# jcmgray/cotengra

Hardware: AMD Instinct MI355X
Metric: contracted FLOP/s (whole node), Sycamore n53 m20 sliced amplitude (higher is better)
Workload: dtype complex64; 1 GPU; Sycamore n53 m20 amplitude, sliced tree, one slice per step per GPU; network=examples/benchmarks/sycamore_n53_m20_s0_e0_pABCDCDAB.json, tree=sycamore_m20_native.json, width_log2=32, parallelism=slice-parallel x1, 1 RCCL reduce, arithmetic=fp16x2 stem pairs and long tiled steps + fp32 MFMA

## Files before the change

### cotengra_amd/csrc/ctg_common.h

```cpp
#pragma once

#include <hip/hip_runtime.h>
#include <cstdlib>
#include <type_traits>
#include <stdint.h>

namespace ctg {

inline bool env_on(const char* name) {
    const char* v = getenv(name);
    return v != nullptr && v[0] != '\0' && !(v[0] == '0' && v[1] == '\0');
}
inline int env_state(const char* name) { return getenv(name) == nullptr ? -1 : (env_on(name) ? 1 : 0); }

inline hipError_t lds_opt_in(const void* kern, int bytes, unsigned long long* done) {
    int dev = 0;
    hipError_t e = hipGetDevice(&dev);
    if (e != hipSuccess) return e;
    const unsigned long long bit = 1ull << (dev & 63);
    if (__atomic_load_n(done, __ATOMIC_ACQUIRE) & bit) return hipSuccess;
    e = hipFuncSetAttribute(kern, hipFuncAttributeMaxDynamicSharedMemorySize, bytes);
    if (e != hipSuccess) {
        (void)hipGetLastError();
        return e;
// ... 58 lines not shown
    void* C;
    const int64_t* soffA;
    const int64_t* soffB;
    const int64_t* soffC;
    int64_t R;
    int64_t Bt;
    int64_t K;
    int64_t N;
    int64_t row_lo;
    int32_t row_lo_shift;
    RowTab rowA, rowB, rowC;
    int64_t k_lo;
    int64_t k_hi_len;
    int32_t k_lo_shift;
    RowTab kA, kB;
    const int64_t* nB;
    const int64_t* nC;
    const int64_t* bA;
    const int64_t* bB;
    const int64_t* bC;
    const double* facA;
    const double* facB;
    int32_t check_zero;
    int32_t nz, z0;
    uint64_t row_lo_magic, k_lo_magic;
    int64_t scratch_total;
    int64_t zA, zB, zC;
    int64_t zsA, zsB, zsC;
    int32_t zqA, zqB;
    int32_t bf3;
};

struct StemArgs {
    const void* A;
    const void* B1;
    const void* B2;
    void* C;
    const int64_t* soffA;
    const int64_t* soffB1;
    const int64_t* soffB2;
    const int64_t* soffC;
    int32_t K1, N1, K2, N2;
    int32_t nr1;
    int32_t rows2;
    int32_t ng2;
    int32_t ld2;
    int64_t n_tiles, g_lo;
    int32_t g_lo_shift;
    int32_t check_zero;
    int32_t vec;
    int32_t bf3;
    const int64_t* gA_hi;
    const int64_t* gA_lo;
    const int64_t* gC_hi;
    const int64_t* gC_lo;
    const int64_t* kj_a;
    const int64_t* lane_a;
    const int64_t* rt_a;
    const int64_t* chunk_a;
    const int64_t* b1_off;
    const int64_t* b2_off;
    const int64_t* mid_row;
    const int64_t* mid_col;
    const int64_t* out_row;
    const int64_t* out_col;
    const double* facA;
    const double* facB1;
    const double* facB2;
    int32_t nz, z0;
    int64_t zA, zB1, zB2, zC;
    int64_t zsA, zsB1, zsB2, zsC;
    int32_t one;
    int32_t tri, KM, NM, rowsM, ngM, ldM;
    const void* BM;
    const int64_t* soffBM;
    const int64_t* bm_off;
    const int64_t* mid2_row;
    const int64_t* mid2_col;
    const double* facBM;
    int64_t zBM, zsBM;
    int64_t a_elems, c_elems;
    const float* amax;
    float* cmax;
};

__device__ __forceinline__ int64_t zid(const StepArgs& p) { return (int64_t)p.z0 + blockIdx.y; }
constexpr int kMaxSub = 16;
__device__ __forceinline__ void record_max(float* slot, float v) {
    atomicMax((unsigned*)slot + ((blockIdx.x + (threadIdx.x >> 6)) & (kMaxSub - 1)), __builtin_bit_cast(unsigned, v));
}
__device__ __forceinline__ float read_max(const float* slot) {
    float m = slot[0];
#pragma unroll
    for (int i = 1; i < kMaxSub; ++i) m = fmaxf(m, slot[i]);
    return m;
}
__device__ __forceinline__ int64_t zgroup(int64_t z, int32_t q) { return q > 1 ? z / q * q : z; }
__device__ __forceinline__ int64_t zoffA(const StepArgs& p) { const int64_t z = zgroup(zid(p), p.zqA); return p.soffA[z * p.zsA] + z * p.zA; }
__device__ __forceinline__ int64_t zoffB(const StepArgs& p) { const int64_t z = zgroup(zid(p), p.zqB); return p.soffB[z * p.zsB] + z * p.zB; }
__device__ __forceinline__ int64_t zoffC(const StepArgs& p) { const int64_t z = zid(p); return p.soffC[z * p.zsC] + z * p.zC; }

__device__ __forceinline__ double step_alpha(const StepArgs& p) {
    if (p.facA == nullptr) return 1.0;
    const double f = (*p.facA) * (*p.facB);
    if (f == 0.0 && p.check_zero) return 0.0;
    return 1.0 / f;
}

template <int I, int N, typename F>
__device__ __forceinline__ void static_for(F&& f) {
    if constexpr (I < N) {
        f(std::integral_constant<int, I>{});
        static_for<I + 1, N>(f);
    }
}

__device__ __forceinline__ int64_t uniform64(int64_t v) {
    const unsigned lo = __builtin_amdgcn_readfirstlane((unsigned)(v & 0xffffffffll));
    const unsigned hi = __builtin_amdgcn_readfirstlane((unsigned)((unsigned long long)v >> 32));
    return (int64_t)(((unsigned long long)hi << 32) | lo);
}

__device__ __forceinline__ float dpp_swap1(float v) {
    return __builtin_bit_cast(float, __builtin_amdgcn_mov_dpp(__builtin_bit_cast(int, v), 0xB1, 0xF, 0xF, true));
}
__device__ __forceinline__ float2 pair_rows(float a_t, float a_t1, bool odd) {
    const float x = dpp_swap1(a_t), y = dpp_swap1(a_t1);
    float2 v;
    v.x = odd ? y : a_t;
    v.y = odd ? a_t1 : x;
    return v;
}
__device__ __forceinline__ float2 pair_rows(float a_t, float a_t1, bool odd, float alpha) {
    const float x = dpp_swap1(a_t), y = dpp_swap1(a_t1);
    float2 v;
    v.x = (odd ? y : a_t) * alpha;
    v.y = (odd ? a_t1 : x) * alpha;
    return v;
}

__device__ __forceinline__ int64_t sload64(const int64_t* p) {
    typedef const int64_t __attribute__((address_space(4))) * cptr;
    return *(cptr)(uintptr_t)p;
}

__device__ __forceinline__ int64_t zoffA_s(const StepArgs& p) { const int64_t z = zgroup(zid(p), p.zqA); return sload64(p.soffA + z * p.zsA) + z * p.zA; }
__device__ __forceinline__ int64_t zoffB_s(const StepArgs& p) { const int64_t z = zgroup(zid(p), p.zqB); return sload64(p.soffB + z * p.zsB) + z * p.zB; }
__device__ __forceinline__ int64_t zoffC_s(const StepArgs& p) { const int64_t z = zid(p); return sload64(p.soffC + z * p.zsC) + z * p.zC; }

__device__ __forceinline__ void split_k(const StepArgs& p, int64_t k, int64_t& hi, int64_t& lo) {
    if (p.k_lo_shift >= 0) {
        hi = k >> p.k_lo_shift;
        lo = k & (p.k_lo - 1);
    } else if (p.k_lo_magic != 0) {
        hi = (int64_t)__umul64hi((uint64_t)k, p.k_lo_magic);
        lo = k - hi * p.k_lo;
    } else {
        hi = k / p.k_lo;
        lo = k - hi * p.k_lo;
    }
}

__device__ __forceinline__ void split_row(const StepArgs& p, int64_t i, int64_t& hi, int64_t& lo) {
    if (p.row_lo_shift >= 0) {
        hi = i >> p.row_lo_shift;
        lo = i & (p.row_lo - 1);
// ... 126 lines not shown

template <typename F>
inline hipError_t for_each_z(const StepArgs& p, F launch_one) {
    if (p.nz <= 1) return launch_one(p);
    for (int z = 0; z < p.nz; ++z) {
        StepArgs q = p;
        q.z0 = p.z0 + z;
        q.nz = 1;
        const hipError_t e = launch_one(q);
        if (e != hipSuccess) return e;
    }
    return hipSuccess;
}

template <typename F>
inline hipError_t for_each_z_chunk(const StepArgs& p, int64_t fit, F launch_chunk) {
    if (fit < 1) fit = 1;
    for (int64_t z = 0; z < p.nz; z += fit) {
        StepArgs q = p;
        q.z0 = p.z0 + (int32_t)z;
        q.nz = (int32_t)(p.nz - z < fit ? p.nz - z : fit);
        const hipError_t e = launch_chunk(q);
        if (e != hipSuccess) return e;
    }
    return hipSuccess;
}


hipError_t launch_pair_valu(int dtype, const StepArgs& p, void* scratch, int64_t scratch_bytes,
                            hipStream_t stream);
struct ValuGroupItem {
    StepArgs p;
    int64_t col_tiles, n_tiles;
    int32_t tn_shift;
    uint32_t block_begin, n_blocks;
};
constexpr int64_t kValuGroupMaxTiles = 4096;
bool valu_thread_per_output(const StepArgs& p);
void pair_valu_name(int dtype, const StepArgs& p, int64_t scratch_bytes, char* buf, size_t n);
uint32_t valu_group_fill(const StepArgs& p, ValuGroupItem* it, uint32_t block_begin);
hipError_t launch_pair_valu_group(int dtype, const ValuGroupItem* d_items, int n_items, uint32_t blocks,
                                  int nz, hipStream_t stream);
hipError_t launch_pair_mfma(int dtype, const StepArgs& p, const MfmaHints& h, void* scratch,
                            int64_t scratch_bytes, hipStream_t stream);
constexpr int64_t kPickKredMinK = 1 << 15, kPickKredMaxM = 512;
inline bool pick_route_kred(int64_t M, int64_t K) { return K >= kPickKredMinK && M <= kPickKredMaxM; }
hipError_t launch_pair_pick(int dtype, const StepArgs& p, int vec, void* scratch, int64_t scratch_bytes,
                            hipStream_t stream);
void pair_pick_name(int dtype, const StepArgs& p, int vec, int64_t scratch_bytes, char* buf, size_t n);
constexpr int64_t kPickRowsMfmaMinRowLo = 32, kPickRowsMfmaMinN = 8, kPickRowsMfmaMinK = 8;
inline bool pick_rows_route_mfma(int64_t row_lo, int64_t K, int64_t N, int dtype) {
    return dtype == 2 && row_lo >= kPickRowsMfmaMinRowLo && N >= kPickRowsMfmaMinN && K >= kPickRowsMfmaMinK;
}
hipError_t launch_pair_pick_rows(int dtype, const StepArgs& p, int vec, int b_fixed, hipStream_t stream);
void pair_pick_rows_name(int dtype, const StepArgs& p, int vec, int b_fixed, char* buf, size_t n);
struct FastGroupItem {
    StepArgs p;
    MfmaHints h;
    int64_t tiles_m, tiles_n;
    uint32_t block_begin, n_blocks;
};
constexpr int64_t kFastGroupMaxTiles = 128;
int fast_group_key(const StepArgs& p, const MfmaHints& h);
uint32_t fast_group_fill(const StepArgs& p, const MfmaHints& h, FastGroupItem* it, uint32_t block_begin);
hipError_t launch_pair_mfma_fast_group(int key, const FastGroupItem* d_items, int n_items, uint32_t blocks,
                                       int nz, hipStream_t stream);
bool rowwise_ok(const StepArgs& p);
void pair_mfma_c64_name(const StepArgs& p, const MfmaHints& h, int64_t scratch_bytes, char* buf, size_t n);
int64_t fast_lane_table_bytes();
hipError_t launch_fast_lane_consts(const StepArgs& p, const MfmaHints& h, void* out, hipStream_t stream);
hipError_t launch_pair_mfma_c128(const StepArgs& p, int flags, hipStream_t stream);
void pair_mfma_c128_name(const StepArgs& p, char* buf, size_t n);
hipError_t launch_pair_mfma_real(int dtype, const StepArgs& p, int flags, hipStream_t stream);
void pair_mfma_real_name(int dtype, const StepArgs& p, int flags, char* buf, size_t n);
bool stem2_supported(const StemArgs& p);
bool stem3_supported(const StemArgs& p);
hipError_t launch_stem2(const StemArgs& p, hipStream_t stream);
void stem2_kernel_name(const StemArgs& p, char* buf, size_t n);
bool stem2h_supported(const StemArgs& p);
bool stem2h_uses_h2(const StemArgs& p);
bool stem2_uses_bf3(const StemArgs& p);
hipError_t launch_stem2h(const StemArgs& p, hipStream_t stream);
void stem2h_kernel_name(const StemArgs& p, char* buf, size_t n);

hipError_t launch_single(int dtype, const StepArgs& p, hipStream_t stream);
bool pair_bf16x3_on(const StepArgs& p);
hipError_t launch_accum(int dtype, const StepArgs& p, const StripState* st, void* wide, const double* inscale, int leaf,
                        hipStream_t stream);
struct AccumGroupItem {
    StepArgs p;
    void* wide;
    int32_t leaf;
    uint32_t block_begin, n_blocks;
};
constexpr int64_t kAccumGroupMaxBlocks = 1 << 16;
uint32_t accum_group_fill(const StepArgs& p, void* wide, int leaf, AccumGroupItem* it, uint32_t block_begin);
hipError_t launch_accum_group(int dtype, const AccumGroupItem* d_items, int n_items, uint32_t blocks, int nz,
                              const double* inscale, hipStream_t stream);
hipError_t launch_prescale_inputs(int dtype, void* inputs, const int64_t* offs, const int64_t* sizes, int64_t n_inputs,
                                  int* shift_total, double* inscale, hipStream_t stream);
hipError_t launch_narrow(int dtype, void* result, const void* wide, int64_t n, hipStream_t stream);
hipError_t launch_widen(int dtype, void* wide, const void* result, int64_t n, hipStream_t stream);

hipError_t launch_maxabs(int dtype, const void* x, int64_t n, double* fac, hipStream_t stream);
hipError_t launch_strip_prepare(const double* fac, const int32_t* counted, int64_t n_steps,
                                int64_t root_step, int check_zero, StripState* st, const double* inscale, hipStream_t stream);
hipError_t launch_rescale(int dtype, void* result, int64_t n, const StripState* st, hipStream_t stream);

struct SliceMeta {
    int64_t n_leaves;
    int64_t n_sliced;
    const int64_t* sizes;
    const int64_t* fixed;
    const int64_t* strides;
    double* fac;
    const int32_t* fac_zero;
    int64_t n_fac;
    float* smax;
    const int32_t* smax_zero;
    int64_t n_smax;
};
hipError_t launch_prologue(const SliceMeta& m, int64_t* state, int64_t* soff, int64_t sid,
                           hipStream_t stream, int nz = 1, int64_t stride = 1, const int64_t* ids = nullptr);
hipError_t launch_set_state(int64_t* state, int64_t next, int64_t stride, hipStream_t stream);

}
```

### cotengra_amd/csrc/ctg_exec_state.h

```cpp
#pragma once

#include <string>
#include <vector>

#include "../../include/ctg_hip.h"
#include "ctg_common.h"
#include "ctg_lds.h"

struct ctg_plan {
    int dtype = 0;
    int64_t n_inputs = 0;
    std::vector<int64_t> input_sizes, input_offsets;
    int64_t inputs_elems = 0, arena_elems = 0, result_elems = 0;
    int64_t n_steps = 0;
    std::vector<int64_t> steps;
    std::vector<int64_t> tables;
    int64_t n_sliced = 0;
    std::vector<int64_t> slice_sizes, slice_fixed, slice_strides;
    std::vector<int64_t> slice_group;
    bool has_groups = false;
    int64_t nslices = 1;
    std::vector<int64_t> max_soff;
};

struct ctg_exec {
    const ctg_plan* plan = nullptr;
    int device = 0;
    hipStream_t stream = nullptr;
    char* d_inputs = nullptr;
    char* d_arena = nullptr;
    char* d_result = nullptr;
    bool owns_result = false;
    char* d_wide = nullptr;
    int64_t* d_in_tab = nullptr;
    double* d_inscale = nullptr;
    int64_t* d_tables = nullptr;
    int64_t* d_misc = nullptr;
    int64_t* d_state = nullptr;
    int64_t* d_zero = nullptr;
    int64_t* d_soff = nullptr;
    void* d_scratch = nullptr;
    ctg::SliceMeta meta{};
    std::vector<ctg::StepArgs> args;
    std::vector<ctg::StemArgs> stem_args;
    int stem_bf16x3 = 1;
    int stem_arith = 2;
    float* d_stem_max = nullptr;
    int32_t* d_smax_zero = nullptr;
    float* smax_slot(int bank, int64_t s, int64_t z) const {
        return d_stem_max + (((int64_t)bank * plan_steps + s) * (batch > 1 ? batch : 1) + z) * ctg::kMaxSub;
    }
    ctg::SliceMeta meta_resetting(int which) const {
        ctg::SliceMeta m = meta;
        if (m.smax) m.smax_zero = d_smax_zero + (int64_t)which * m.n_smax;
        return m;
    }
    int64_t plan_steps = 0;
    std::vector<char> rec_wanted;
    std::vector<char> wave_member;
    std::vector<char> stem_h2_ran;
    std::vector<ctg::MfmaHints> hints;
    std::vector<ctg::MfmaHints> hints_b;
    uint16_t* d_ord_b = nullptr;
    char* d_lane_b = nullptr;
    uint16_t* d_ord = nullptr;
    char* d_lane = nullptr;
    int batch = 1;
    int group_d = 0;
    int64_t* d_batch_ids = nullptr;
    int64_t* h_ids = nullptr;
    size_t h_ids_cap = 0;
    hipEvent_t ev_ids = nullptr;
    int batch_nominal = 1;
    int64_t scratch_total = 0;
    struct Issue {
        int64_t step;
        int cls;
        int32_t item0, n;
        uint32_t blocks;
        bool shared = false;
    };
    std::vector<Issue> issue;
    std::vector<Issue> issue_reuse;
    std::vector<int32_t> lds_comp_of;
    int lds_first[2] = {0, 0}, lds_count[2] = {0, 0}, lds_bytes[2] = {0, 0};
    ctg::LdsCompDev* d_lds_comps = nullptr;
    char* d_lds_blob = nullptr;
    ctg::ValuGroupItem* d_group_items = nullptr;
    ctg::AccumGroupItem* d_accum_items = nullptr;
    std::vector<char> accum_member;
    ctg::FastGroupItem* d_fast_items = nullptr;
    std::vector<hipEvent_t> events;
    hipStream_t gstream = nullptr;
    hipGraphExec_t gexec = nullptr;
    hipEvent_t ev_in = nullptr, ev_out = nullptr;
    bool warm = false;
    bool soff_static = false;
    bool graph_off = false;
    int strip = 0, check_zero = 0;
    double* d_fac = nullptr;
    int32_t* d_counted = nullptr;
    int32_t* d_fac_zero = nullptr;
    std::vector<char> invariant;
    bool invariants_ready = false;
    std::vector<char> grouped;
    int64_t group_key = -1;
    ctg::StripState* d_strip = nullptr;
    int64_t root_step = -1;
    void* d_sample_blocks = nullptr;
    void* d_sample_io = nullptr;
    int64_t sample_blocks_bytes = 0, sample_io_bytes = 0;
    double sample_last[4] = {0, 0, 0, 0};
    float sample_pass_ms[2] = {0, 0};
    bool sample_last_valid = false;
    hipEvent_t sample_ev[3] = {nullptr, nullptr, nullptr};
    void* d_range = nullptr;
    int64_t range_bytes = 0;
    void* d_reduce = nullptr;
    int64_t reduce_bytes = 0;
};


inline int64_t ctg_item_size(int dtype) {
    static const int64_t k[4] = {4, 8, 8, 16};
    return k[dtype];
}

extern "C" __attribute__((visibility("hidden"))) void ctg_set_error_(const char* msg);

namespace ctg {
hipError_t launch_maxabs_f32(const void* base, const int64_t* soff, int64_t z, int64_t zs, int64_t zstride, int64_t n,
                             float* out, hipStream_t stream, int nz = 1, int out_zs = 0);
}

namespace ctg {
constexpr int64_t kRangeMaxBlocks = 2048;
constexpr int64_t kRangeMaxComponents = 1ll << 40;
int64_t range_blocks(int64_t n);
int64_t range_partial_bytes(int64_t blocks);
hipError_t launch_range_hist(const void* x, int64_t n, void* partials, int64_t blocks, int64_t* row, double* sumsq,
                             hipStream_t stream);
}
// ... 22 lines not shown
```

### cotengra_amd/csrc/ctg_runtime.hip

```cpp
#include <algorithm>
#include <cstdarg>
#include <cmath>
#include <cstdio>
#include <cstdlib>
#include <cstring>
#include <string>
#include <vector>

#include "ctg_exec_state.h"

using namespace ctg;

namespace {

thread_local std::string g_err;

int fail(int code, const char* fmt, ...) {
    char buf[1024];
    va_list ap;
    va_start(ap, fmt);
    vsnprintf(buf, sizeof(buf), fmt, ap);
    va_end(ap);
    g_err = buf;
    return code;
// ... 72 lines not shown
        return fail(CTG_E_INVALID, "step %lld: bad stem grid", sl);
    const int64_t rows1 = 1ll << nr1;
    const int64_t len[ST_COUNT] = {n_tiles / g_lo, g_lo, n_tiles / g_lo, g_lo, 8, 64, rows1 / 32, K1 / 16,
                                   K1 * N1, one ? 1 : K2 * N2, one ? 1 : rows1, one ? 1 : N1,
                                   one ? rows1 : rows2, one ? N1 : N2};
    int64_t mx[ST_COUNT], mn[ST_COUNT];
    for (int t = 0; t < ST_COUNT; ++t) {
        if (!tab_ok(p, h[SW_TABS + t], len[t]))
            return fail(CTG_E_BOUNDS, "step %lld: stem table outside the blob", sl);
        mx[t] = tab_max(p, h[SW_TABS + t], len[t], &mn[t]);
        if (mn[t] < 0) return fail(CTG_E_BOUNDS, "step %lld: negative stem offset", sl);
    }
    if (mx[ST_LANE_A] >= (1ll << 29))
        return fail(CTG_E_INVALID, "step %lld: stem lane offsets beyond 32 bits", sl);
    if (h[SW_VEC] != 0 && h[SW_VEC] != 1) return fail(CTG_E_INVALID, "step %lld: bad stem gather mode", sl);
    if (h[SW_VEC]) {
        const int64_t* kj = &p->tables[h[SW_TABS + ST_KJ_A]];
        for (int q = 0; q < 4; ++q)
            if (kj[2 * q + 1] != kj[2 * q] + 1 || (kj[2 * q] & 1))
                return fail(CTG_E_INVALID, "step %lld: stem slots not paired for 16-byte gathers", sl);
        const int odd_tabs[5] = {ST_GA_HI, ST_GA_LO, ST_LANE_A, ST_RT_A, ST_CHUNK_A};
        for (int t : odd_tabs)
            for (int64_t i = 0; i < len[t]; ++i)
                if (p->tables[h[SW_TABS + t] + i] & 1)
                    return fail(CTG_E_INVALID, "step %lld: odd stem offset under 16-byte gathers", sl);
        if ((r[W_A_OFF] & 1) || r[W_A_LEAF] >= 0)
            return fail(CTG_E_INVALID, "step %lld: stem operand not aligned for 16-byte gathers", sl);
    }
    if (h[SW_TRI] != 0 && h[SW_TRI] != 1) return fail(CTG_E_INVALID, "step %lld: bad stem stage count", sl);
    const bool tri = h[SW_TRI] == 1;
    int64_t bm_top = 0;
    if (tri) {
        const int64_t KM = h[SW_KM], NM = h[SW_NM], rowsM = h[SW_ROWSM];
        if (one || KM < 16 || KM > 128 || NM < 16 || NM > 128 || rowsM < 32 || rowsM > (1 << 16) ||
            h[SW_LDM] != KM + 4 || rows1 * N1 != rowsM * KM || rowsM * NM != rows2 * K2)
            return fail(CTG_E_INVALID, "step %lld: three-step tile shape the kernel does not take", sl);
        a.tri = 1; a.KM = (int)KM; a.NM = (int)NM; a.rowsM = (int)rowsM; a.ngM = (int)h[SW_NGM]; a.ldM = (int)h[SW_LDM];
        a.vec = (int)h[SW_VEC];
        if (!stem3_supported(a))
            return fail(CTG_E_INVALID, "step %lld: three-step tile shape the kernel does not take", sl);
        const int64_t lenm[3] = {KM * NM, rowsM, NM};
        int64_t mxm[3], mnm[3];
        for (int t = 0; t < 3; ++t) {
            if (!tab_ok(p, h[SW_TABS_M + t], lenm[t]))
                return fail(CTG_E_BOUNDS, "step %lld: stem table outside the blob", sl);
            mxm[t] = tab_max(p, h[SW_TABS_M + t], lenm[t], &mnm[t]);
            if (mnm[t] < 0) return fail(CTG_E_BOUNDS, "step %lld: negative stem offset", sl);
        }
        bm_top = mxm[0];
        if (mx[ST_MID_ROW] + mx[ST_MID_COL] >= rowsM * (KM + 4) || mxm[1] + mxm[2] >= rows2 * (K2 + 4))
            return fail(CTG_E_BOUNDS, "step %lld: intermediate tile overflows its LDS", sl);
        const int64_t cap = space_elems(p, h[SW_BM_SPACE]);
        if (cap < 0) return fail(CTG_E_INVALID, "step %lld: bad space", sl);
        if (h[SW_BM_LEAF] < -1 || h[SW_BM_LEAF] > p->n_inputs) return fail(CTG_E_INVALID, "step %lld: bad leaf", sl);
        const int64_t hi = h[SW_BM_OFF] + (h[SW_BM_LEAF] >= 0 ? p->max_soff[h[SW_BM_LEAF]] : 0) + bm_top;
        if (h[SW_BM_OFF] < 0 || hi >= cap)
            return fail(CTG_E_BOUNDS, "step %lld: stem operand m reaches element %lld of a space of %lld", sl,
                        (long long)hi, (long long)cap);
    }
    if (!one && !tri && mx[ST_MID_ROW] + mx[ST_MID_COL] >= rows2 * (K2 + 4))
        return fail(CTG_E_BOUNDS, "step %lld: intermediate tile overflows its LDS", sl);
    struct Op { int64_t space, off, leaf, size, top; char name; };
    const Op ops[4] = {
        {r[W_A_SPACE], r[W_A_OFF], r[W_A_LEAF], r[W_A_SIZE],
         mx[ST_GA_HI] + mx[ST_GA_LO] + mx[ST_RT_A] + mx[ST_CHUNK_A] + mx[ST_KJ_A] + mx[ST_LANE_A], 'A'},
        {r[W_B_SPACE], r[W_B_OFF], r[W_B_LEAF], r[W_B_SIZE], mx[ST_B1_OFF], 'B'},
        {h[SW_B2_SPACE], h[SW_B2_OFF], h[SW_B2_LEAF], h[SW_B2_SIZE], mx[ST_B2_OFF], 'b'},
        {r[W_C_SPACE], r[W_C_OFF], r[W_C_LEAF], r[W_C_SIZE],
         mx[ST_GC_HI] + mx[ST_GC_LO] + mx[ST_OUT_ROW] + mx[ST_OUT_COL], 'C'},
    };
    for (const Op& op : ops) {
        if (one && op.name == 'b') continue;
        const int64_t cap = space_elems(p, op.space);
        if (cap < 0) return fail(CTG_E_INVALID, "step %lld: bad space", sl);
        if (op.leaf < -1 || op.leaf > p->n_inputs) return fail(CTG_E_INVALID, "step %lld: bad leaf", sl);
        if (op.name == 'C' && op.space == SPACE_INPUTS)
            return fail(CTG_E_INVALID, "step %lld: writes into the inputs space", sl);
        const int64_t hi = op.off + (op.leaf >= 0 ? p->max_soff[op.leaf] : 0) + op.top;
        if (op.off < 0 || hi >= cap)
            return fail(CTG_E_BOUNDS, "step %lld: stem operand %c reaches element %lld of a space of %lld",
                        sl, op.name, (long long)hi, (long long)cap);
    }
    return CTG_OK;
}

int validate_plan(ctg_plan* p) {
    if (p->dtype < 0 || p->dtype > 3) return fail(CTG_E_INVALID, "bad dtype %d", p->dtype);
    if (p->n_inputs < 1) return fail(CTG_E_INVALID, "plan needs at least one input");
    for (int64_t i = 0; i < p->n_inputs; ++i) {
        if (p->input_sizes[i] < 1 || p->input_offsets[i] < 0 ||
            p->input_offsets[i] + p->input_sizes[i] > p->inputs_elems)
            return fail(CTG_E_BOUNDS, "input %lld does not fit the inputs space", (long long)i);
    }
    p->nslices = 1;
    p->max_soff.assign(p->n_inputs + 1, 0);
    for (int64_t j = 0; j < p->n_sliced; ++j) {
        const int64_t d = p->slice_sizes[j], f = p->slice_fixed[j];
        if (d < 1) return fail(CTG_E_INVALID, "bad slice size");
        if (f >= 0 && d != 1) return fail(CTG_E_INVALID, "projected index must have size 1");
        p->nslices = (p->nslices > INT64_MAX / d) ? INT64_MAX : p->nslices * d;
        for (int64_t l = 0; l <= p->n_inputs; ++l) {
            const int64_t st = p->slice_strides[l * p->n_sliced + j];
            if (st < 0) return fail(CTG_E_INVALID, "negative slice stride");
            p->max_soff[l] += st * (f >= 0 ? f : d - 1);
        }
    }
    bool any_group = false;
    for (int64_t j = 0; j < p->n_sliced; ++j) {
        const int64_t g = p->slice_group[j];
        if (g != 0 && g != 1) return fail(CTG_E_INVALID, "bad slice group flag");
        if (g == 1 && p->slice_fixed[j] >= 0) return fail(CTG_E_INVALID, "a projected index cannot be a group index");
        any_group = any_group || g == 1;
    }
    p->has_groups = false;
    for (int64_t s = 0; s < p->n_steps; ++s) {
        const int64_t* r = &p->steps[s * STEP_WORDS];
        const int64_t kind = r[W_KIND];
        if (kind < 0 || kind > 3) return fail(CTG_E_INVALID, "step %lld: bad kind", (long long)s);
        if (r[W_INVARIANT] < 0 || r[W_INVARIANT] > 2 || (r[W_INVARIANT] == 2 && !any_group))
            return fail(CTG_E_INVALID, "step %lld: bad sharing class", (long long)s);
        p->has_groups = p->has_groups || (r[W_INVARIANT] == 2 && kind != KIND_ACCUM);
        if (kind == KIND_STEM2) {
            const int rc = validate_stem(p, s);
            if (rc != CTG_OK) return rc;
            continue;
        }
        if (r[W_KERNEL] < 0 || r[W_KERNEL] > 3)
            return fail(CTG_E_INVALID, "step %lld: bad kernel", (long long)s);
        if (r[W_KERNEL] == KERNEL_PICK_ROWS && (kind != KIND_PAIR || r[W_BT] != 1))
            return fail(CTG_E_INVALID, "step %lld: the pick rows kernel executes pair steps with Bt = 1 only", (long long)s);
        if (r[W_KERNEL] == KERNEL_PICK_ROWS)
            for (int w : {W_ROWA_HI, W_ROWA_LO, W_ROWB_HI, W_ROWB_LO, W_ROWC_HI, W_ROWC_LO, W_KA_HI, W_KA, W_KB_HI,
                          W_KB, W_NB, W_NC})
                if (r[w] < 0)
                    return fail(CTG_E_INVALID, "step %lld: the pick rows kernel needs every row, k and n table", (long long)s);
        if (r[W_KERNEL] == KERNEL_PICK && (kind != KIND_PAIR || r[W_N] != 1 || r[W_BT] != 1 || r[W_ROW_LO] != 1))
            return fail(CTG_E_INVALID, "step %lld: the pick kernel executes pair steps with N = 1, Bt = 1 and row_lo = 1 only",
                        (long long)s);
        if (r[W_KERNEL] == KERNEL_PICK)
            for (int w : {W_ROWA_HI, W_ROWA_LO, W_ROWB_HI, W_ROWB_LO, W_ROWC_HI, W_ROWC_LO, W_KA_HI, W_KA, W_KB_HI,
                          W_KB, W_NB, W_NC})
                if (r[w] < 0)
                    return fail(CTG_E_INVALID, "step %lld: the pick kernel needs every row, k and n table", (long long)s);
        if (r[W_KERNEL] == KERNEL_MFMA && kind != KIND_PAIR)
            return fail(CTG_E_INVALID, "step %lld: the matrix-core kernels execute pair steps only",
                        (long long)s);
        const int64_t R = r[W_R], Bt = r[W_BT], K = r[W_K], N = r[W_N];
        const int64_t row_lo = r[W_ROW_LO], row_hi = r[W_ROW_HI_LEN];
        const int64_t k_lo = r[W_K_LO], k_hi = r[W_K_HI_LEN];
        if (R < 1 || Bt < 1 || K < 1 || N < 1 || row_lo < 1 || row_hi < 1 || k_lo < 1 || k_hi < 1)
            return fail(CTG_E_INVALID, "step %lld: non-positive extent", (long long)s);
        if (row_lo * row_hi != R) return fail(CTG_E_INVALID, "step %lld: row split != R", (long long)s);
        if (k_lo * k_hi != K) return fail(CTG_E_INVALID, "step %lld: k split != K", (long long)s);
        if (r[W_KERNEL] == KERNEL_MFMA && Bt > 65535)
            return fail(CTG_E_INVALID, "step %lld: MFMA batch too large", (long long)s);

        struct Op { int space_w, off_w, leaf_w, size_w; int64_t rhi, rlo, khi, klo, n, b; bool used; };
        const bool pair = kind == KIND_PAIR, mfma = r[W_KERNEL] == KERNEL_MFMA;
        Op ops[3] = {
            {W_A_SPACE, W_A_OFF, W_A_LEAF, W_A_SIZE, r[W_ROWA_HI], r[W_ROWA_LO],
             kind != KIND_ACCUM ? r[W_KA_HI] : -1, kind != KIND_ACCUM ? r[W_KA] : -1, -1,
             mfma ? r[W_BA] : -1, true},
            {W_B_SPACE, W_B_OFF, W_B_LEAF, W_B_SIZE, mfma ? -1 : r[W_ROWB_HI], mfma ? -1 : r[W_ROWB_LO],
             r[W_KB_HI], r[W_KB], r[W_NB], mfma ? r[W_BB] : -1, pair},
            {W_C_SPACE, W_C_OFF, W_C_LEAF, W_C_SIZE, r[W_ROWC_HI], r[W_ROWC_LO], -1, -1,
             pair ? r[W_NC] : -1, mfma ? r[W_BC] : -1, true},
// ... 164 lines not shown
        auto magic = [](int64_t d, int64_t range) -> uint64_t {
            if (d < 2 || (d & (d - 1)) == 0 || range + 4096 >= (1ll << 32)) return 0;
            return (uint64_t)(~0ull / (uint64_t)d) + 1;
        };
        a.row_lo_magic = magic(a.row_lo, r[W_R]);
        a.rowA = RowTab{tab(W_ROWA_HI), tab(W_ROWA_LO)};
        a.rowB = RowTab{tab(W_ROWB_HI), tab(W_ROWB_LO)};
        a.rowC = RowTab{tab(W_ROWC_HI), tab(W_ROWC_LO)};
        a.k_lo = r[W_K_LO];
        a.k_hi_len = r[W_K_HI_LEN];
        a.k_lo_shift = log2_exact(a.k_lo);
        a.k_lo_magic = magic(a.k_lo, r[W_K]);
        a.kA = RowTab{tab(W_KA_HI), tab(W_KA)};
        a.kB = RowTab{tab(W_KB_HI), tab(W_KB)};
        a.nB = tab(W_NB);
        a.nC = tab(W_NC);
        a.bA = tab(W_BA);
        a.bB = tab(W_BB);
        a.bC = tab(W_BC);
        a.nz = 1;
        a.z0 = 0;
        a.scratch_total = e->scratch_total;
        a.zA = per_slice(r[W_A_SPACE], r[W_A_OFF]);
        a.zB = per_slice(r[W_B_SPACE], r[W_B_OFF]);
        a.zC = per_slice(r[W_C_SPACE], r[W_C_OFF]);
        a.zsA = r[W_A_LEAF] >= 0 ? p->n_inputs + 1 : 0;
        a.zsB = r[W_B_LEAF] >= 0 ? p->n_inputs + 1 : 0;
        a.zsC = r[W_C_LEAF] >= 0 ? p->n_inputs + 1 : 0;
        if (e->group_d > 1) {
            auto shared = [&](int64_t st) {
                return st >= 0 && st < p->n_steps && p->steps[st * STEP_WORDS + W_INVARIANT] == 2 &&
                       p->steps[st * STEP_WORDS + W_KIND] != KIND_ACCUM;
            };
            const int64_t d = e->group_d;
            if (shared(s)) {
                a.zA *= d; a.zB *= d; a.zC *= d;
                a.zsA *= d; a.zsB *= d; a.zsC *= d;
            } else if (r[W_KIND] == KIND_PAIR || r[W_KIND] == KIND_SINGLE) {
                auto writer = [&](int sw, int ow) -> int64_t {
                    if (r[sw] != SPACE_ARENA) return -1;
                    for (int64_t t = s - 1; t >= 0; --t) {
                        const int64_t* w = &p->steps[t * STEP_WORDS];
                        if (w[W_KIND] != KIND_ACCUM && w[W_C_SPACE] == SPACE_ARENA && w[W_C_OFF] == r[ow]) return t;
                    }
                    return -1;
                };
                if (shared(writer(W_A_SPACE, W_A_OFF))) a.zqA = (int32_t)d;
                if (r[W_KIND] == KIND_PAIR && shared(writer(W_B_SPACE, W_B_OFF))) a.zqB = (int32_t)d;
            }
        }
        a.facA = a.facB = nullptr;
        a.check_zero = e->check_zero;
        a.bf3 = e->stem_bf16x3;
        if (e->strip && r[W_KIND] == KIND_PAIR) {
            auto fac = [&](int w) -> const double* {
                return (r[w] >= 0 && r[w] < p->n_steps) ? e->d_fac + r[w] : e->d_fac + p->n_steps;
            };
            a.facA = fac(W_A_PROD);
            a.facB = fac(W_B_PROD);
        }
        if (r[W_KIND] == KIND_STEM2) {
            const int64_t* h = &p->tables[r[W_STEM]];
            StemArgs& q = e->stem_args[s];
            memset(&q, 0, sizeof(q));
            q.A = a.A;
            q.B1 = a.B;
            q.C = a.C;
            q.one = h[SW_ONE] == 1 ? 1 : 0;
            q.B2 = q.one ? nullptr : (char*)space_ptr(e, h[SW_B2_SPACE]) + h[SW_B2_OFF] * isz;
            q.soffA = a.soffA;
            q.soffB1 = a.soffB;
            q.soffC = a.soffC;
            q.soffB2 = h[SW_B2_LEAF] >= 0 ? e->d_soff + h[SW_B2_LEAF] : e->d_zero;
            q.K1 = (int)h[SW_K1]; q.N1 = (int)h[SW_N1]; q.K2 = (int)h[SW_K2]; q.N2 = (int)h[SW_N2];
            q.nr1 = (int)h[SW_NR1]; q.rows2 = (int)h[SW_ROWS2]; q.ng2 = (int)h[SW_NG2]; q.ld2 = (int)h[SW_LD2];
            q.n_tiles = h[SW_NTILES];
            q.g_lo = h[SW_GLO];
            q.g_lo_shift = log2_exact(q.g_lo);
            q.check_zero = e->check_zero;
            q.vec = (int)h[SW_VEC];
            q.bf3 = e->stem_bf16x3;
            q.a_elems = r[W_A_SIZE];
            q.c_elems = r[W_C_SIZE];
            const int64_t** tabs[ST_COUNT] = {&q.gA_hi, &q.gA_lo, &q.gC_hi, &q.gC_lo, &q.kj_a, &q.lane_a, &q.rt_a,
                                              &q.chunk_a, &q.b1_off, &q.b2_off, &q.mid_row, &q.mid_col,
                                              &q.out_row, &q.out_col};
            for (int t = 0; t < ST_COUNT; ++t) *tabs[t] = T + h[SW_TABS + t];
            q.nz = 1;
            q.z0 = 0;
            q.zA = a.zA; q.zB1 = a.zB; q.zC = a.zC;
            q.zB2 = per_slice(h[SW_B2_SPACE], h[SW_B2_OFF]);
            q.zsA = a.zsA; q.zsB1 = a.zsB; q.zsC = a.zsC;
            q.zsB2 = h[SW_B2_LEAF] >= 0 ? p->n_inputs + 1 : 0;
            if (e->strip) {
                auto fac = [&](int64_t w) -> const double* {
                    return (w >= 0 && w < p->n_steps) ? e->d_fac + w : e->d_fac + p->n_steps;
                };
                q.facA = fac(r[W_A_PROD]);
                q.facB1 = fac(r[W_B_PROD]);
                q.facB2 = q.one ? e->d_fac + p->n_steps : fac(h[SW_B2_PROD]);
                q.facBM = h[SW_TRI] == 1 ? fac(h[SW_BM_PROD]) : e->d_fac + p->n_steps;
            }
            if (h[SW_TRI] == 1) {
                q.tri = 1;
                q.KM = (int)h[SW_KM]; q.NM = (int)h[SW_NM]; q.rowsM = (int)h[SW_ROWSM]; q.ngM = (int)h[SW_NGM];
                q.ldM = (int)h[SW_LDM];
                q.BM = (char*)space_ptr(e, h[SW_BM_SPACE]) + h[SW_BM_OFF] * isz;
                q.soffBM = h[SW_BM_LEAF] >= 0 ? e->d_soff + h[SW_BM_LEAF] : e->d_zero;
                q.bm_off = T + h[SW_TABS_M];
                q.mid2_row = T + h[SW_TABS_M + 1];
                q.mid2_col = T + h[SW_TABS_M + 2];
                q.zBM = per_slice(h[SW_BM_SPACE], h[SW_BM_OFF]);
                q.zsBM = h[SW_BM_LEAF] >= 0 ? p->n_inputs + 1 : 0;
            }
        }
    }
}


int64_t tab2(const ctg_plan* p, int64_t hi_w, int64_t lo_w, int64_t lo_size, int64_t i) {
    return p->tables[hi_w + i / lo_size] + p->tables[lo_w + i % lo_size];
}

bool tile_additive(const ctg_plan* p, int64_t lo_w, int64_t lo_size, int64_t total, int B) {
    if (total % B) return false;
    if (lo_size % B) return false;
    for (int64_t t = 0; t < lo_size / B; ++t)
        for (int r = 0; r < B; ++r)
            if (p->tables[lo_w + t * B + r] - p->tables[lo_w + t * B] != p->tables[lo_w + r])
                return false;
    return true;
}

bool all_even(const ctg_plan* p, int64_t w, int64_t len, int64_t stride = 1) {
    for (int64_t i = 0; i < len; i += stride)
        if (p->tables[w + i] & 1) return false;
    return true;
}

bool pick_vec_ok(const ctg_plan* p, const int64_t* r) {
    const int64_t k_lo = r[W_K_LO];
    if ((k_lo & 1) || (r[W_A_OFF] & 1) || (r[W_B_OFF] & 1)) return false;
    for (int64_t i = 0; i < k_lo; ++i)
        if (p->tables[r[W_KA] + i] != i || p->tables[r[W_KB] + i] != i) return false;
    if (!all_even(p, r[W_KA_HI], r[W_K_HI_LEN]) || !all_even(p, r[W_KB_HI], r[W_K_HI_LEN])) return false;
    if (!all_even(p, r[W_ROWA_HI], r[W_ROW_HI_LEN]) || !all_even(p, r[W_ROWB_HI], r[W_ROW_HI_LEN])) return false;
    if (!all_even(p, r[W_ROWA_LO], r[W_ROW_LO]) || !all_even(p, r[W_ROWB_LO], r[W_ROW_LO]) || !all_even(p, r[W_NB], r[W_N]))
        return false;
    if (p->arena_elems & 1) return false;
    for (int lw : {W_A_LEAF, W_B_LEAF})
        if (r[lw] >= 0)
            for (int64_t j = 0; j < p->n_sliced; ++j)
                if (p->slice_strides[r[lw] * p->n_sliced + j] & 1) return false;
    return true;
}

void build_mfma_order(const ctg_plan* p, const int64_t* r, int bn, int BM,
                      std::vector<uint16_t>& blob, size_t* offA, size_t* offB, int* vecA,
                      int TB = 256) {
    const int BK = MFMA_BK;
    const int T = BM == 32 ? 64 : 256;
    const int64_t R = r[W_R], K = r[W_K], N = r[W_N];
    const int64_t BIG = INT64_MAX / 4;
    {
        const int n_el = BM * BK, per_t = n_el / T;
        std::vector<int64_t> off(n_el);
// ... 454 lines not shown
    if (ev1) (void)hipEventDestroy(ev1);
}

static bool tiled16_step(const ctg_exec* e, int64_t s) {
    const ctg_plan* p = e->plan;
    const int64_t* r = &p->steps[s * STEP_WORDS];
    if (r[W_KIND] != KIND_PAIR || r[W_KERNEL] != KERNEL_MFMA || p->dtype != CTG_C64) return false;
    const MfmaHints& h = e->hints[s];
    return !h.stream && h.fast && h.bf3 && e->stem_arith != 0 && !e->strip && e->d_stem_max != nullptr &&
           pair_bf16x3_on(e->args[s]);
}

static bool stem_step_h2(const ctg_exec* e, int64_t s, bool recorded) {
    return e->stem_arith == 2 && !e->strip && e->d_stem_max != nullptr && (recorded || env_on("CTG_STEM_H2_ALL")) &&
           stem2h_uses_h2(e->stem_args[s]) && env_state("CTG_STEM_H2") != 0;
}
static bool pair_step_h2(const ctg_exec* e, bool single) {
    return e->stem_arith == 2 && single && env_state("CTG_PAIR_H2") != 0;
}

static bool pair_records(const ctg_exec* e, int64_t s) {
    const ctg_plan* p = e->plan;
    const int64_t* r = &p->steps[s * STEP_WORDS];
    if (r[W_KIND] != KIND_PAIR || r[W_KERNEL] != KERNEL_MFMA || p->dtype != CTG_C64) return false;
    if (e->stem_arith == 0 || e->strip || e->d_stem_max == nullptr || e->grouped[s]) return false;
    const MfmaHints& h = e->hints[s];
    if (tiled16_step(e, s)) return h.splitk <= 1 && e->args[s].zqA <= 1 && e->args[s].zqB <= 1;
    if (e->stem_arith != 2 || e->wave_member[s] || !e->rec_wanted[s]) return false;
    return h.stream == 1 || (!h.stream && h.fast && !h.bf3 && h.splitk <= 1);
}

int launch_step(ctg_exec* e, int64_t s, hipStream_t stream) {
    const ctg_plan* p = e->plan;
    const int64_t* r = &p->steps[s * STEP_WORDS];
    hipError_t err = hipSuccess;
    if (!e->d_scratch && step_needs_scratch(e, s)) {
        const int rc = ensure_scratch(e);
        if (rc != CTG_OK) return rc;
    }
    switch (r[W_KIND]) {
        case KIND_SINGLE: err = launch_single(p->dtype, e->args[s], stream); break;
        case KIND_ACCUM:
            if (e->strip) {
                err = launch_strip_prepare(e->d_fac, e->d_counted, p->n_steps, e->root_step,
                                           e->check_zero, e->d_strip, e->d_inscale, stream);
                if (err == hipSuccess)
                    err = launch_rescale(p->dtype, e->d_result, p->result_elems, e->d_strip, stream);
                if (err == hipSuccess && e->d_wide)
                    err = launch_rescale(p->dtype + 1, e->d_wide, p->result_elems, e->d_strip, stream);
                if (err == hipSuccess) err = launch_accum(p->dtype, e->args[s], e->d_strip, wide_of_step(e, s), nullptr, -1, stream);
            } else {
                err = launch_accum(p->dtype, e->args[s], nullptr, wide_of_step(e, s), e->d_inscale, accum_leaf(p, s), stream);
            }
            break;
        case KIND_STEM2: {
            const int nz = e->args[s].nz;
            const bool rec = e->stem_arith != 0 && !e->strip && e->d_stem_max != nullptr;
            const int64_t prod = r[W_A_PROD];
            const bool prod_rec = prod >= 0 && prod < p->n_steps && e->stem_h2_ran[prod];
            const bool h2 = stem_step_h2(e, s, prod_rec);
            const bool records = h2 || (rec && stem2_uses_bf3(e->stem_args[s]));
            e->stem_h2_ran[s] = records ? 1 : 0;
            if (env_on("CTG_STEM_DEBUG"))
                fprintf(stderr, "stem step %lld: arith %d rec %d prod %lld prod_rec %d uses_h2 %d uses_bf3 %d -> h2 %d records %d\n",
                        (long long)s, e->stem_arith, (int)rec, (long long)prod, (int)prod_rec, (int)stem2h_uses_h2(e->stem_args[s]),
                        (int)stem2_uses_bf3(e->stem_args[s]), (int)h2, (int)records);
            for (int z = 0; z < nz && err == hipSuccess; ++z) {
                StemArgs q = e->stem_args[s];
                q.z0 = e->args[s].z0 + z;
                q.nz = 1;
                const int64_t zc = (e->invariant[s] || e->grouped[s]) ? 0 : q.z0;
                const int64_t za = (prod_rec && (e->invariant[prod] || e->grouped[prod])) ? 0 : q.z0;
                q.amax = h2 ? e->smax_slot(0, prod_rec ? prod : 0, za) : nullptr;
                q.cmax = records ? e->smax_slot(0, s, zc) : nullptr;
                if (h2 && !prod_rec) {
                    float* slot = e->smax_slot(1, s, q.z0);
                    err = hipMemsetAsync(slot, 0, sizeof(float) * kMaxSub, stream);
                    if (err == hipSuccess)
                        err = r[W_A_LEAF] >= 0 ? launch_maxabs_f32(q.A, nullptr, 0, 0, 0, q.a_elems, slot, stream)
                                               : launch_maxabs_f32(q.A, q.soffA, q.z0, q.zsA, q.zA, q.a_elems, slot, stream);
                    q.amax = slot;
                }
                if (err == hipSuccess) err = h2 ? launch_stem2h(q, stream) : launch_stem2(q, stream);
            }
            break;
        }
        case KIND_PAIR:
            if (r[W_KERNEL] == KERNEL_MFMA && p->dtype == CTG_C128)
                err = launch_pair_mfma_c128(e->args[s], e->hints[s].vecA , stream);
            else if (r[W_KERNEL] == KERNEL_MFMA && p->dtype != CTG_C64)
                err = launch_pair_mfma_real(p->dtype, e->args[s], e->hints[s].vecA, stream);
            else if (r[W_KERNEL] == KERNEL_MFMA) {
                const MfmaHints& h0 = (e->args[s].nz > 1 && !e->hints_b.empty()) ? e->hints_b[s] : e->hints[s];
                const bool tiled16 = tiled16_step(e, s) && !h0.stream && h0.fast && h0.bf3;
                if (tiled16) {
                    MfmaHints h = h0;
                    const StepArgs& a = e->args[s];
                    const bool single = h0.splitk <= 1 && a.zqA <= 1 && a.zqB <= 1 && !e->grouped[s] &&
                                        a.z0 + a.nz <= std::max(e->batch, 1);
                    const bool h2 = pair_step_h2(e, single);
                    h.h2 = h2 ? 1 : 0;
                    h.cmax = single ? e->smax_slot(0, s, 0) : nullptr;
                    h.cmax_zs = e->invariant[s] ? 0 : 1;
                    e->stem_h2_ran[s] = single ? 1 : 0;
                    for (int side = 0; side < 2 && h2 && err == hipSuccess; ++side) {
                        const int64_t prod = r[side == 0 ? W_A_PROD : W_B_PROD];
                        const float* mx = nullptr;
                        int zs = 1;
                        if (prod >= 0 && prod < p->n_steps && e->stem_h2_ran[prod] && !e->grouped[prod]) {
                            mx = e->smax_slot(0, prod, 0);
                            zs = e->invariant[prod] ? 0 : 1;
                        } else if (r[side == 0 ? W_A_LEAF : W_B_LEAF] >= 0) {
                            float* slot = e->smax_slot(1 + side, s, 0);
                            err = hipMemsetAsync(slot, 0, sizeof(float) * kMaxSub, stream);
                            if (err == hipSuccess)
                                err = launch_maxabs_f32(side == 0 ? a.A : a.B, nullptr, 0, 0, 0, r[side == 0 ? W_A_SIZE : W_B_SIZE], slot, stream);
                            mx = slot;
                            zs = 0;
                        } else {
                            float* slot = e->smax_slot(1 + side, s, 0);
                            float* at = slot + (int64_t)a.z0 * kMaxSub;
                            err = hipMemsetAsync(at, 0, sizeof(float) * kMaxSub * (size_t)a.nz, stream);
                            if (err == hipSuccess)
                                err = side == 0 ? launch_maxabs_f32(a.A, a.soffA, a.z0, a.zsA, a.zA, r[W_A_SIZE], at, stream, a.nz, kMaxSub)
                                                : launch_maxabs_f32(a.B, a.soffB, a.z0, a.zsB, a.zB, r[W_B_SIZE], at, stream, a.nz, kMaxSub);
                            mx = slot;
                        }
                        (side == 0 ? h.amax : h.bmax) = mx;
                        (side == 0 ? h.amax_zs : h.bmax_zs) = zs;
                    }
                    if (env_on("CTG_STEM_DEBUG"))
                        fprintf(stderr, "tiled step %lld: arith %d single %d -> h2 %d records %d (A prod %lld, B prod %lld)\n",
                                (long long)s, e->stem_arith, (int)single, (int)h2, (int)single, (long long)r[W_A_PROD],
                                (long long)r[W_B_PROD]);
                    if (err == hipSuccess) err = launch_pair_mfma(p->dtype, e->args[s], h, e->d_scratch, kScratchBytes, stream);
                } else {
                    const StepArgs& a = e->args[s];
                    const bool can = e->stem_arith == 2 && !e->strip && e->d_stem_max != nullptr && !e->grouped[s] &&
                                     !env_on("CTG_NO_PAIR_RECORD") &&
                                     !e->wave_member[s] && e->rec_wanted[s] && a.z0 + a.nz <= std::max(e->batch, 1) &&
                                     ((h0.stream == 1) || (!h0.stream && h0.fast && !h0.bf3 && h0.splitk <= 1));
                    if (!e->stem_h2_ran.empty()) e->stem_h2_ran[s] = can ? 1 : 0;
                    if (can) {
                        MfmaHints h = h0;
                        h.cmax = e->smax_slot(0, s, 0);
                        h.cmax_zs = e->invariant[s] ? 0 : 1;
                        err = launch_pair_mfma(p->dtype, a, h, e->d_scratch, kScratchBytes, stream);
                    } else {
                        err = launch_pair_mfma(p->dtype, a, h0, e->d_scratch, kScratchBytes, stream);
                    }
                }
            } else if (r[W_KERNEL] == KERNEL_PICK)
                err = launch_pair_pick(p->dtype, e->args[s], e->hints[s].vecA, e->d_scratch, kScratchBytes, stream);
            else if (r[W_KERNEL] == KERNEL_PICK_ROWS)
                err = launch_pair_pick_rows(p->dtype, e->args[s], e->hints[s].vecA, e->hints[s].fast, stream);
            else
                err = launch_pair_valu(p->dtype, e->args[s], e->d_scratch, kScratchBytes, stream);
            break;
    }
    if (err == hipSuccess && e->strip && (r[W_KIND] == KIND_PAIR || r[W_KIND] == KIND_STEM2)) {
        const char* c = (const char*)space_ptr(e, r[W_C_SPACE]) + r[W_C_OFF] * kItemSize[p->dtype];
        err = launch_maxabs(p->dtype, c, r[W_C_SIZE], e->d_fac + s, stream);
    }
    if (err != hipSuccess)
        return fail(CTG_E_HIP, "launch of step %lld failed: %s", (long long)s, hipGetErrorString(err));
    return CTG_OK;
// ... 528 lines not shown
        std::vector<double> init(3 + (p->n_inputs + 1) / 2, 0.0);
        init[0] = 1.0;
        HIP_TRY_E(hipMalloc((void**)&e->d_inscale, init.size() * sizeof(double)));
        HIP_TRY_E(hipMemcpy(e->d_inscale, init.data(), init.size() * sizeof(double), hipMemcpyHostToDevice));
    }
    {
        bool sums = false;
        for (int64_t s = 0; s < p->n_steps; ++s) sums = sums || p->steps[s * STEP_WORDS + W_KIND] == KIND_ACCUM;
        sums = sums && p->nslices > 1;
        if (sums && (p->dtype == CTG_F32 || p->dtype == CTG_C64) && !env_on("CTG_NO_WIDE_SUM")) {
            HIP_TRY_E(hipMalloc((void**)&e->d_wide, p->result_elems * 2 * isz));
            HIP_TRY_E(hipMemsetAsync(e->d_wide, 0, p->result_elems * 2 * isz, e->stream));
        }
    }
    HIP_TRY_E(hipMalloc((void**)&e->d_tables, p->tables.size() * 8));
    e->scratch_total = kScratchBytes * std::min<int64_t>(std::max(e->batch, 1), 8);
    const int64_t n_leaves = p->n_inputs + 1;
    const int64_t misc_words = 3 + n_leaves * e->batch + 2 * p->n_sliced + n_leaves * p->n_sliced + e->batch;
    HIP_TRY_E(hipMalloc((void**)&e->d_misc, misc_words * 8));
    std::vector<int64_t> misc(misc_words, 0);
    int64_t* cur = e->d_misc;
    e->d_state = cur;
    cur += 2;
    e->d_zero = cur;
    cur += 1;
    e->d_soff = cur;
    cur += n_leaves * e->batch;
    int64_t* d_sizes = cur;
    cur += p->n_sliced;
    int64_t* d_fixed = cur;
    cur += p->n_sliced;
    int64_t* d_strides = cur;
    e->d_batch_ids = d_strides + n_leaves * p->n_sliced;
    for (int64_t j = 0; j < p->n_sliced; ++j) {
        misc[(d_sizes - e->d_misc) + j] = p->slice_sizes[j];
        misc[(d_fixed - e->d_misc) + j] = p->slice_fixed[j];
    }
    for (int64_t i = 0; i < n_leaves * p->n_sliced; ++i)
        misc[(d_strides - e->d_misc) + i] = p->slice_strides[i];
    misc[1] = 1;
    HIP_TRY_E(hipMemcpy(e->d_misc, misc.data(), misc_words * 8, hipMemcpyHostToDevice));
    HIP_TRY_E(hipMemcpy(e->d_tables, p->tables.data(), p->tables.size() * 8, hipMemcpyHostToDevice));
    HIP_TRY_E(hipMemsetAsync(e->d_inputs, 0, p->inputs_elems * isz, e->stream));
    HIP_TRY_E(hipMemsetAsync(e->d_result, 0, p->result_elems * isz, e->stream));
    e->meta = SliceMeta{n_leaves, p->n_sliced, d_sizes, d_fixed, d_strides, nullptr, nullptr, 0, nullptr, nullptr, 0};
    {
        std::vector<double> fac(p->n_steps + 1, 0.0);
        fac[p->n_steps] = 1.0;
        std::vector<int32_t> counted(std::max<int64_t>(p->n_steps, 1), 0);
        std::vector<int32_t> fac_zero(std::max<int64_t>(p->n_steps, 1), 0);
        e->invariant.assign(p->n_steps, 0);
        e->grouped.assign(p->n_steps, 0);
        for (int64_t st = 0; st < p->n_steps; ++st)
            e->grouped[st] = p->has_groups && p->steps[st * STEP_WORDS + W_INVARIANT] == 2 &&
                             p->steps[st * STEP_WORDS + W_KIND] != KIND_ACCUM;
        for (int64_t st = 0; st < p->n_steps; ++st) {
            const int64_t* r = &p->steps[st * STEP_WORDS];
            e->invariant[st] = r[W_INVARIANT] == 1 && r[W_KIND] != KIND_ACCUM;
            if (r[W_KIND] == KIND_PAIR || r[W_KIND] == KIND_STEM2) {
                counted[st] = 1;
                fac_zero[st] = e->invariant[st] ? 0 : 1;
                e->root_step = st;
            }
        }
        {
            bool stems = false;
            const int64_t nb = std::max<int64_t>(e->batch, 1);
            e->plan_steps = p->n_steps;
            const size_t bank = (size_t)(std::max<int64_t>(p->n_steps, 1) * nb * kMaxSub);
            std::vector<int32_t> sz(3 * bank, 0);
            for (int64_t st = 0; st < p->n_steps; ++st) {
                const int64_t* rs = &p->steps[st * STEP_WORDS];
                stems = stems || rs[W_KIND] == KIND_STEM2;
                const bool can = rs[W_KIND] == KIND_STEM2 || (rs[W_KIND] == KIND_PAIR && rs[W_KERNEL] == KERNEL_MFMA);
                if (!can) continue;
                for (int64_t z = 0; z < nb * kMaxSub; ++z) {
                    const size_t at = (size_t)(st * nb * kMaxSub + z);
                    sz[at] = e->invariant[st] ? 0 : 1;
                    sz[bank + at] = (e->invariant[st] || e->grouped[st]) ? 0 : 1;
                    sz[2 * bank + at] = 1;
                }
            }
            e->stem_h2_ran.assign(p->n_steps, 0);
            if (e->wave_member.size() != (size_t)p->n_steps) e->wave_member.assign(p->n_steps, 0);
            (void)stems;
            if (p->dtype == CTG_C64) {
                HIP_TRY_E(hipMalloc((void**)&e->d_stem_max, sz.size() * sizeof(float)));
                HIP_TRY_E(hipMemset(e->d_stem_max, 0, sz.size() * sizeof(float)));
                HIP_TRY_E(hipMalloc((void**)&e->d_smax_zero, sz.size() * sizeof(int32_t)));
                HIP_TRY_E(hipMemcpy(e->d_smax_zero, sz.data(), sz.size() * sizeof(int32_t), hipMemcpyHostToDevice));
                e->meta.smax = e->d_stem_max;
                e->meta.smax_zero = e->d_smax_zero;
                e->meta.n_smax = (int64_t)(sz.size() / 3);
            }
        }
        HIP_TRY_E(hipMalloc((void**)&e->d_fac_zero, fac_zero.size() * sizeof(int32_t)));
        HIP_TRY_E(hipMemcpy(e->d_fac_zero, fac_zero.data(), fac_zero.size() * sizeof(int32_t),
                            hipMemcpyHostToDevice));
        HIP_TRY_E(hipMalloc((void**)&e->d_fac, fac.size() * sizeof(double)));
        HIP_TRY_E(hipMalloc((void**)&e->d_counted, counted.size() * sizeof(int32_t)));
        HIP_TRY_E(hipMalloc((void**)&e->d_strip, sizeof(StripState)));
        HIP_TRY_E(hipMemcpy(e->d_fac, fac.data(), fac.size() * sizeof(double), hipMemcpyHostToDevice));
        HIP_TRY_E(hipMemcpy(e->d_counted, counted.data(), counted.size() * sizeof(int32_t),
                            hipMemcpyHostToDevice));
    }
    e->graph_off = !env_on("CTG_GRAPH");
    if (const char* v = getenv("CTG_STEM_ARITH")) {
        const std::string a(v);
        if (a == "fp32" || a == "0") e->stem_arith = 0;
        else if (a == "bf16x3" || a == "1") e->stem_arith = 1;
        else if (a == "fp16x2" || a == "2") e->stem_arith = 2;
        e->stem_bf16x3 = e->stem_arith ? 1 : 0;
    }
    resolve_args(e);
    {
        int rc = build_hints(e);
        if (rc == CTG_OK) rc = build_groups(e);
        for (int64_t st = 0; rc == CTG_OK && st < p->n_steps; ++st)
            if (step_needs_scratch(e, st)) {
                rc = ensure_scratch(e);
                break;
            }
        if (rc != CTG_OK) return bail(rc);
    }
    *out = e;
    return CTG_OK;
#undef HIP_TRY_E
}

int ctg_exec_set_stream(ctg_exec* e, void* stream) {
    if (!e) return fail(CTG_E_INVALID, "null argument");
    if ((hipStream_t)stream == e->stream) return CTG_OK;
    HIP_TRY(hipSetDevice(e->device));
    HIP_TRY(hipStreamSynchronize(e->stream));
    e->stream = (hipStream_t)stream;
    return CTG_OK;
}

int ctg_exec_upload_inputs_host(ctg_exec* e, const void* const* ptrs) {
    if (!e || !ptrs) return fail(CTG_E_INVALID, "null argument");
    HIP_TRY(hipSetDevice(e->device));
    const ctg_plan* p = e->plan;
    const int64_t isz = kItemSize[p->dtype];
    std::vector<char> staging((size_t)(p->inputs_elems * isz), 0);
    for (int64_t i = 0; i < p->n_inputs; ++i) {
        if (!ptrs[i]) return fail(CTG_E_INVALID, "input %lld is null", (long long)i);
        memcpy(staging.data() + p->input_offsets[i] * isz, ptrs[i], p->input_sizes[i] * isz);
    }
    HIP_TRY(hipStreamSynchronize(e->stream));
    HIP_TRY(hipMemcpy(e->d_inputs, staging.data(), staging.size(), hipMemcpyHostToDevice));
    if (e->d_inscale)
        HIP_TRY(launch_prescale_inputs(p->dtype, e->d_inputs, e->d_in_tab, e->d_in_tab + p->n_inputs, p->n_inputs,
                                       (int*)(e->d_inscale + 2), e->d_inscale, e->stream));
    e->invariants_ready = false;
    e->group_key = -1;
    return CTG_OK;
}

int ctg_exec_upload_inputs_device(ctg_exec* e, const void* const* ptrs) {
    if (!e || !ptrs) return fail(CTG_E_INVALID, "null argument");
    HIP_TRY(hipSetDevice(e->device));
    const ctg_plan* p = e->plan;
    const int64_t isz = kItemSize[p->dtype];
    for (int64_t i = 0; i < p->n_inputs; ++i) {
        if (!ptrs[i]) return fail(CTG_E_INVALID, "input %lld is null", (long long)i);
        HIP_TRY(hipMemcpyAsync(e->d_inputs + p->input_offsets[i] * isz, ptrs[i],
// ... 434 lines not shown
        if (rc != CTG_OK) return rc;
    }
    {
        const int rc = run_invariants(e);
        if (rc != CTG_OK) return rc;
    }
    for (int64_t s = 0; s < p->n_steps; ++s) {
        if (!e->invariant[s] || !audited(s)) continue;
        const int64_t* r = &p->steps[s * STEP_WORDS];
        const int rc = pass(e->d_arena, r[W_C_OFF], r[W_C_SIZE], p->arena_elems, p->n_inputs + s);
        if (rc != CTG_OK) return rc;
    }
    hipError_t err = launch_prologue(e->meta, e->d_state, e->d_soff, slice_id, e->stream, 1, 1);
    if (err != hipSuccess) return fail(CTG_E_HIP, "prologue launch failed: %s", hipGetErrorString(err));
    bool lds_done[2] = {false, false};
    for (int64_t s = 0; s < p->n_steps; ++s) {
        if (e->invariant[s]) continue;
        if (!e->lds_comp_of.empty() && e->lds_comp_of[s] >= 0) {
            const int cls = e->grouped[s] ? 0 : 1;
            if (!lds_done[cls] && p->steps[s * STEP_WORDS + W_KIND] == KIND_PAIR) {
                lds_done[cls] = true;
                const ctg_exec::Issue q{s, -2, e->lds_first[cls], e->lds_count[cls], (uint32_t)e->lds_count[cls], cls == 0};
                const int rc = launch_issue(e, q, 1, e->stream);
                if (rc != CTG_OK) return rc;
            }
            continue;
        }
        {
            const int rc = launch_step(e, s, e->stream);
            if (rc != CTG_OK) return rc;
        }
        if (!audited(s)) continue;
        const int64_t* r = &p->steps[s * STEP_WORDS];
        const int rc = pass(e->d_arena, r[W_C_OFF], r[W_C_SIZE], p->arena_elems, p->n_inputs + s);
        if (rc != CTG_OK) return rc;
    }
    HIP_TRY(hipMemcpyAsync(rows, d_rows, (size_t)rows_bytes, hipMemcpyDeviceToHost, e->stream));
    HIP_TRY(hipMemcpyAsync(sumsq, d_sumsq, (size_t)(T * 8), hipMemcpyDeviceToHost, e->stream));
    HIP_TRY(hipStreamSynchronize(e->stream));
    return CTG_OK;
}

int ctg_exec_step_kernel(ctg_exec* e, int64_t step, char* buf, int64_t buflen) {
    if (!e || !buf || buflen < 1) return fail(CTG_E_INVALID, "null argument");
    const ctg_plan* p = e->plan;
    if (step < 0 || step >= p->n_steps) return fail(CTG_E_INVALID, "step out of range");
    const int64_t* r = &p->steps[step * STEP_WORDS];
    char name[128];
    if (!e->lds_comp_of.empty() && e->lds_comp_of[step] >= 0) {
        snprintf(name, sizeof(name), "lds_run_kernel[%d]", (int)e->lds_comp_of[step]);
    } else if (r[W_KIND] == KIND_SINGLE) {
        snprintf(name, sizeof(name), "single_kernel");
    } else if (r[W_KIND] == KIND_ACCUM) {
        snprintf(name, sizeof(name), (size_t)step < e->accum_member.size() && e->accum_member[step] ? "accum_group_kernel"
                                                                                                    : "accum_kernel");
    } else if (r[W_KIND] == KIND_STEM2) {
        const int64_t prod = r[W_A_PROD];
        const bool prod16 = prod >= 0 && prod < p->n_steps &&
                            ((p->steps[prod * STEP_WORDS + W_KIND] == KIND_STEM2 &&
                              (stem2_uses_bf3(e->stem_args[prod]) || stem2h_uses_h2(e->stem_args[prod]))) ||
                             pair_records(e, prod));
        if (stem_step_h2(e, step, prod16)) stem2h_kernel_name(e->stem_args[step], name, sizeof(name));
        else stem2_kernel_name(e->stem_args[step], name, sizeof(name));
    } else if (r[W_KERNEL] == KERNEL_MFMA && p->dtype == CTG_C128) {
        pair_mfma_c128_name(e->args[step], name, sizeof(name));
    } else if (r[W_KERNEL] == KERNEL_MFMA && p->dtype != CTG_C64) {
        pair_mfma_real_name(p->dtype, e->args[step], e->hints[step].vecA, name, sizeof(name));
    } else if (r[W_KERNEL] == KERNEL_MFMA) {
        MfmaHints h = e->hints[step];
        h.h2 = pair_step_h2(e, tiled16_step(e, step) && h.splitk <= 1 && !e->grouped[step] &&
                                   e->args[step].zqA <= 1 && e->args[step].zqB <= 1) ? 1 : 0;
        pair_mfma_c64_name(e->args[step], h, kScratchBytes, name, sizeof(name));
    } else if (r[W_KERNEL] == KERNEL_PICK) {
        pair_pick_name(p->dtype, e->args[step], e->hints[step].vecA, kScratchBytes, name, sizeof(name));
    } else if (r[W_KERNEL] == KERNEL_PICK_ROWS) {
        pair_pick_rows_name(p->dtype, e->args[step], e->hints[step].vecA, e->hints[step].fast, name, sizeof(name));
    } else {
        pair_valu_name(p->dtype, e->args[step], kScratchBytes, name, sizeof(name));
    }
    snprintf(buf, (size_t)buflen, "%s", name);
    return CTG_OK;
}

int ctg_exec_sync(ctg_exec* e) {
    if (!e) return fail(CTG_E_INVALID, "null argument");
    HIP_TRY(hipSetDevice(e->device));
    HIP_TRY(hipStreamSynchronize(e->stream));
    return CTG_OK;
}

int ctg_exec_result_ptr(ctg_exec* e, void** dev_ptr) {
    if (!e || !dev_ptr) return fail(CTG_E_INVALID, "null argument");
    *dev_ptr = e->d_result;
    return CTG_OK;
}

int ctg_exec_download_result(ctg_exec* e, void* host_out) {
    if (!e || !host_out) return fail(CTG_E_INVALID, "null argument");
    HIP_TRY(hipSetDevice(e->device));
    HIP_TRY(hipStreamSynchronize(e->stream));
    HIP_TRY(hipMemcpy(host_out, e->d_result, e->plan->result_elems * kItemSize[e->plan->dtype],
                      hipMemcpyDeviceToHost));
    return CTG_OK;
}

int ctg_exec_download_arena(ctg_exec* e, int64_t offset, int64_t n, void* host_out) {
    if (!e || !host_out) return fail(CTG_E_INVALID, "null argument");
    if (offset < 0 || n < 0 || offset + n > e->plan->arena_elems)
        return fail(CTG_E_BOUNDS, "arena range out of bounds");
    const int64_t isz = kItemSize[e->plan->dtype];
    HIP_TRY(hipSetDevice(e->device));
    HIP_TRY(hipStreamSynchronize(e->stream));
    HIP_TRY(hipMemcpy(host_out, e->d_arena + offset * isz, n * isz, hipMemcpyDeviceToHost));
    return CTG_OK;
}

}
```

### cotengra_amd/csrc/ctg_stem.hip

```cpp
#include "ctg_stem_impl.h"

namespace ctg {
#ifdef CTG_STEM_DEV_ONE
template __global__ void stem2_kernel<CTG_STEM_DEV_ONE>(StemArgs);
#else
bool stem2_supported(const StemArgs& p) { return stem2_supported_shape(p); }
bool stem3_supported(const StemArgs& p) { return stem3_supported_shape(p); }
bool stem2_uses_bf3(const StemArgs& p) { return stem_uses_16bit(p); }
void stem2_kernel_name(const StemArgs& p, char* buf, size_t n) { stem_kernel_name<Bf16x3>(p, buf, n); }
hipError_t launch_stem2(const StemArgs& p, hipStream_t stream) { return launch_stem<Bf16x3>(p, stream); }
#endif
}

#ifndef CTG_STEM_DEV_ONE
extern "C" int ctg_stem_triple_instantiated(int p1, int pm, int p2, int rt1, int cs1, int nch, int itm, int it2, int vec) {
    return ctg::stem3_instantiated(p1 != 0, pm != 0, p2 != 0, rt1, cs1, nch, itm, it2, vec != 0) ? 1 : 0;
}
#endif
#ifdef CTG_STEM_TIMELINE
extern "C" int ctg_debug_stem_timeline(unsigned long long* out, int reset) { return ctg::stem_debug_timeline<ctg::Bf16x3>(out, reset); }
#endif
#ifdef CTG_STEM_BOUNDS
extern "C" int ctg_debug_stem_oob(unsigned long long out[2], int reset) { return ctg::stem_debug_oob<ctg::Bf16x3>(out, reset); }
#endif
```

### cotengra_amd/csrc/ctg_stem_h2.hip

```cpp
#include "ctg_stem_impl.h"

namespace ctg {
#ifdef CTG_STEM_DEV_ONE
template __global__ void stem2h_kernel<CTG_STEM_DEV_ONE>(StemArgs);
#else
bool stem2h_supported(const StemArgs& p) { return stem2_supported_shape(p); }
bool stem2h_uses_h2(const StemArgs& p) { return stem_uses_16bit(p); }
void stem2h_kernel_name(const StemArgs& p, char* buf, size_t n) { stem_kernel_name<Fp16x2>(p, buf, n); }
hipError_t launch_stem2h(const StemArgs& p, hipStream_t stream) { return launch_stem<Fp16x2>(p, stream); }
#endif
}

#ifdef CTG_STEM_TIMELINE
extern "C" int ctg_debug_stem_timeline_h2(unsigned long long* out, int reset) { return ctg::stem_debug_timeline<ctg::Fp16x2>(out, reset); }
#endif
#ifdef CTG_STEM_BOUNDS
extern "C" int ctg_debug_stem_oob_h2(unsigned long long out[2], int reset) { return ctg::stem_debug_oob<ctg::Fp16x2>(out, reset); }
#endif
```

### cotengra_amd/csrc/ctg_stem_impl.h

```cpp
#pragma once
#include "ctg_common.h"

#include <cstdio>
#include <cstdlib>
#include <type_traits>


namespace ctg {

typedef float f32x16 __attribute__((ext_vector_type(16)));
typedef float f32x4 __attribute__((ext_vector_type(4)));

#ifdef CTG_STEM_BOUNDS
template <class AR>
__device__ unsigned long long ctg_stem_oob[2];
#endif

#ifdef CTG_STEM_TIMELINE
#define CTG_TL_TILES 256
template <class AR>
__device__ unsigned long long ctg_stem_tl[8][CTG_TL_TILES][6];
template <class AR>
__device__ int ctg_stem_tl_on;
#endif
// ... 135 lines not shown
                                                  int N, int planes, int tid, bool vec, float scale) {
    const int ROW = bf3_row(K, STEP1);
    for (int e = tid; e < K * N; e += SW * 64) {
        const int k = e / N, n = e - k * N;
        int at;
        if (STEP1) {
            const int h = vec ? (k >> 1) & 1 : k & 1;
            const int slot = vec ? (((k & 15) >> 2) << 1) | (k & 1) : (k & 15) >> 1;
            at = (k >> 4) * 48 + h * 24 + slot;
        } else {
            at = (k >> 3) * 24 + (k & 7);
        }
        const c64 v = B[off[e]];
        const float vals[3] = {v.re * scale, v.im * scale, -v.im * scale};
#pragma unroll
        for (int pl = 0; pl < 3; ++pl) {
            if (pl >= planes) break;
            AR::store_limbs(Q + (pl * N + n) * ROW + at, vals[pl]);
        }
    }
}

template <class AR>
__device__ __forceinline__ int bf3_operand_exponent(const c64* __restrict__ B, const int64_t* off, int n_el, int tid,
                                                    float* red) {
    float mx = 0.f;
    for (int e = tid; e < n_el; e += SW * 64) {
        const c64 v = B[off[e]];
        mx = fmaxf(mx, fmaxf(fabsf(v.re), fabsf(v.im)));
    }
#pragma unroll
    for (int o = 32; o > 0; o >>= 1) mx = fmaxf(mx, __shfl_xor(mx, o));
    if ((tid & 63) == 0) red[tid >> 6] = mx;
    __syncthreads();
    mx = red[0];
#pragma unroll
    for (int w = 1; w < SW; ++w) mx = fmaxf(mx, red[w]);
    __syncthreads();
    return AR::operand_exponent(mx);
}
__device__ __forceinline__ int h2_exponent_of(float mx) {
    const int ex = (int)((__builtin_bit_cast(unsigned, mx) >> 23) & 255u) - 127;
    if (mx == 0.f || ex == 128 || ex == -127) return 0;
    const int e = ex - 13;
    return e < -126 ? -126 : (e > 126 ? 126 : e);
}
__device__ __forceinline__ float pow2f(int ex) {
    return __builtin_bit_cast(float, (unsigned)(ex + 127) << 23);
}

}

#ifdef CTG_STEM_TIMELINE
#define CTG_TL_STAMP(k)                                                                                   \
    do {                                                                                                  \
        if (blockIdx.x == 0 && lane == 0 && tl_n < CTG_TL_TILES && ctg_stem_tl_on<AR>)                    \
            ctg_stem_tl<AR>[wave][tl_n][k] = __builtin_readcyclecounter();                                \
        if ((k) == 5) ++tl_n;                                                                             \
    } while (0)
#else
#define CTG_TL_STAMP(k) do {} while (0)
#endif

template <typename T>
__device__ __forceinline__ void settle(T& v) {
    asm volatile("" : "+v"(v));
}

#ifndef CTG_STEM_WS_DEPTH
#define CTG_STEM_WS_DEPTH 2
#endif
#ifndef CTG_STEM_DEPTH
#define CTG_STEM_DEPTH 2
#endif
#ifndef CTG_STEM_GATHER_PORTIONS
#define CTG_STEM_GATHER_PORTIONS 1
#endif
#ifndef CTG_STEM_NT_STORES
#define CTG_STEM_NT_STORES 1
#endif
constexpr bool STEM_NT_STORES = CTG_STEM_NT_STORES != 0;
constexpr bool STEM_GATHER_PORTIONS = CTG_STEM_GATHER_PORTIONS != 0;
template <class AR, bool PACK1, bool PACK2, int RT1_, int CS1, int NCH, int IT2_, bool BR1, int K2Q, bool VEC, bool BF3,
          bool RI2, bool ONE, int ITM, bool PACKM, bool XM, bool LM, bool WS>
__device__ __forceinline__ void stem2_body(const StemArgs& p) {
    constexpr bool TRI = ITM > 0;
    static_assert(!LM, "reserved (the limb intermediate was removed): kernel names stay 17 arguments long");
    static_assert(BF3 || !AR::fp16, "fp16 x 2: the 16-bit kernels only (its object has no fp32 products)");
    static_assert(!AR::fp16 || !TRI, "fp16 x 2: pairs and single steps");
    static_assert(!WS || (XM && !ONE && IT2_ > 0 && IT2_ <= 2 && (PACK1 || RT1_ == 1)), "specialised waves: a static 16-bit pair");
    constexpr int PW = WS ? 4 : SW;
    constexpr int RT1 = WS ? 2 * RT1_ : RT1_;
    constexpr int IT2 = WS ? 2 * IT2_ : IT2_;
    static_assert(!XM || (BF3 && !TRI && NCH > 0), "two-accumulator real part: bf16 x 3, static, no three-step tile");
    constexpr bool XM1 = XM && !PACK1 && !WS;
    constexpr bool XM2 = XM && !PACK2;
    static_assert(!TRI || (NCH > 0 && IT2 > 0 && !RI2 && !ONE && K2Q == 0), "three-step tile: static, X / Y form");
    static_assert(!ONE || (!PACK1 && !PACK2 && !RI2 && IT2 == 0 && K2Q == 0), "one step: >= 32 columns, nothing of step 2");
    static_assert(!PACK1 || CS1 == 1, "16 columns are one group");
    static_assert(!BR1 || NCH > 0, "B1 in registers needs the chunk count at compile time");
    static_assert(K2Q == 0 || PACK2 || IT2 == 1 || RI2, "B2 in registers: one column group per wave");
    static_assert(!RI2 || (!PACK2 && !BF3 && NCH > 0 && IT2 > 0), "row-interleaved step 2: fp32, >= 32 columns, static");
    constexpr bool SH1 = WS && CS1 > 1 && RT1 % CS1 == 0;
    constexpr int CG1 = SH1 ? CS1 : 1;
    constexpr int RR1 = RT1 / CG1;
    constexpr int RTW = SH1 ? PW : PW / CS1;
    constexpr bool STATIC = NCH > 0;
    extern __shared__ __attribute__((aligned(16))) char smem[];
    const int K1 = p.K1, N1 = p.N1, K2 = K2Q > 0 ? 4 * K2Q : p.K2, N2 = p.N2;
    const int LDB1 = K1 + 4, LDB2 = K2 + 4, LD2 = K2Q > 0 ? 4 * K2Q + 4 : p.ld2;
    const int PLANE = p.rows2 * LD2;
    const int KM = TRI ? p.KM : 0, NM = TRI ? p.NM : 0, LDM = TRI ? p.ldM : 0, LDBM = KM + 4;
    const int PLANEM = TRI ? p.rowsM * LDM : 0;
    const int PLANE1 = TRI ? PLANEM : PLANE;
    float* P1 = (float*)smem;
    float* PM = P1 + (PACK1 ? 3 : 2) * N1 * LDB1;
    float* P2 = PM + (TRI ? (PACKM ? 3 : 2) * NM * LDBM : 0);
    float* mid = P2 + (PACK2 ? 3 : 2) * N2 * LDB2;
    const int RP = 3 * LD2;
    auto ri_off = [&](int e) __attribute__((always_inline)) { return RI2 ? (e / LD2) * RP + e % LD2 : e; };
    int mid_floats = 2 * (PLANE > PLANEM ? PLANE : PLANEM);
    if constexpr (RI2) {
        mid_floats = 3 * PLANE;
        if constexpr (K2Q > 0) {
            mid = P2;
            const int p2f = 2 * N2 * LDB2;
            mid_floats = mid_floats > p2f ? mid_floats : p2f;
        }
    }
    const int ROW1 = bf3_row(K1, true), ROW2 = bf3_row(K2, false), ROWM = TRI ? bf3_row(KM, false) : 0;
    unsigned short* Q1 = (unsigned short*)smem;
    unsigned short* QM = Q1 + (PACK1 ? 3 : 2) * N1 * ROW1;
    unsigned short* Q2 = QM + (TRI ? (PACKM ? 3 : 2) * NM * ROWM : 0);
    if constexpr (BF3) mid = (float*)(Q2 + (PACK2 ? 3 : 2) * N2 * ROW2);
    int64_t* oc_s = (int64_t*)(mid + ((mid_floats + 1) & ~1));

    const int tid = threadIdx.x;
    const int lane = tid & 63;
    const int wave = __builtin_amdgcn_readfirstlane(tid >> 6);
    const int kk = lane >> 5;
    const int l31 = lane & 31;
    const bool producer = !WS || wave < PW;
    const int wave1 = WS ? (wave & (PW - 1)) : wave;
    const int wrt = SH1 ? wave1 : wave1 / CS1;
    const int wcol = SH1 ? 0 : (wave1 % CS1) * 32;

    const int64_t z = (int64_t)p.z0 + blockIdx.y;
    const c64* __restrict__ A = (const c64*)p.A + (sload64(p.soffA + z * p.zsA) + z * p.zA);
    const c64* __restrict__ B1 = (const c64*)p.B1 + (sload64(p.soffB1 + z * p.zsB1) + z * p.zB1);
    const c64* __restrict__ B2 = (const c64*)p.B2 + (sload64(p.soffB2 + z * p.zsB2) + z * p.zB2);
    float* __restrict__ C = (float*)((c64*)p.C + (sload64(p.soffC + z * p.zsC) + z * p.zC));
    const c64* __restrict__ BM = TRI ? (const c64*)p.BM + (sload64(p.soffBM + z * p.zsBM) + z * p.zBM) : nullptr;

    int bf3_ex = 0;
    float* const bf3_red = (float*)(oc_s + (ONE ? N1 : N2));
    float h2_sa = 1.f;
    int h2_exa = 0;
    if constexpr (AR::fp16) {
        h2_exa = p.amax != nullptr ? h2_exponent_of(read_max(p.amax)) : 0;
        h2_exa = __builtin_amdgcn_readfirstlane(h2_exa);
        h2_sa = pow2f(-h2_exa);
    }
    float h2_st = 1.f;
    float h2_vmax = 0.f;
    if constexpr (BF3) {
        const int ex1 = bf3_operand_exponent<AR>(B1, p.b1_off, K1 * N1, tid, bf3_red);
        const int ex2 = ONE ? 0 : bf3_operand_exponent<AR>(B2, p.b2_off, K2 * N2, tid, bf3_red);
        int exm = 0;
        if constexpr (TRI) {
// ... 215 lines not shown
    int64_t pend0 = 0, pend1 = 0, pend2 = 0, pend3 = 0;
    bool pend_live = false;
    auto prep = [&](auto always_tag) __attribute__((always_inline)) {
        constexpr bool ALWAYS = decltype(always_tag)::value;
        pend_live = ALWAYS || ig < n_tiles;
        if (pend_live) {
            const int64_t g = ALWAYS ? (ig < last_tile ? ig : last_tile) : ig;
            const int64_t gh = g >> p.g_lo_shift, gl = g & (p.g_lo - 1);
            pend0 = sload64(p.gA_hi + uniform64(gh));
            pend1 = sload64(p.gA_lo + uniform64(gl));
            pend2 = sload64(p.rt_a + (wrt + RTW * im));
            pend3 = sload64(p.chunk_a + ic);
            if (++ic == nch) {
                ic = 0;
                if (++im == RR1) {
                    im = 0;
                    ig += tile_step;
                }
            }
        }
    };
    auto fire2 = [&](c64 (&r)[8], int q, int64_t base, auto always_tag) __attribute__((always_inline)) {
        if (decltype(always_tag)::value || pend_live) {
            if constexpr (XM) {
                typedef const __attribute__((address_space(1))) char* gptr;
                uint64_t u0 = (uint64_t)A + ((uint64_t)(base + kj[2 * q]) << 3);
                uint64_t u1 = (uint64_t)A + ((uint64_t)(base + kj[2 * q + 1]) << 3);
                asm volatile("" : "+s"(u0), "+s"(u1));
                settle(a_lane);
                const unsigned al = a_lane;
                if (VEC) {
                    const f32x4 v = *(const __attribute__((address_space(1))) f32x4*)((gptr)u0 + al);
                    r[2 * q] = c64{v[0], v[1]};
                    r[2 * q + 1] = c64{v[2], v[3]};
                } else {
                    typedef float f32x2 __attribute__((ext_vector_type(2)));
                    const f32x2 v0 = *(const __attribute__((address_space(1))) f32x2*)((gptr)u0 + al);
                    const f32x2 v1 = *(const __attribute__((address_space(1))) f32x2*)((gptr)u1 + al);
                    r[2 * q] = c64{v0[0], v0[1]};
                    r[2 * q + 1] = c64{v1[0], v1[1]};
                }
                return;
            }
            const char* sb = (const char*)(A + (base + kj[2 * q]));
#ifdef CTG_STEM_BOUNDS
            {
                const uint64_t lim = (uint64_t)p.a_elems * 8;
                const uint64_t o0 = (uint64_t)(sb + a_lane - (const char*)A);
                const uint64_t o1 = VEC ? o0 + 8 : (uint64_t)((const char*)(A + (base + kj[2 * q + 1])) + a_lane - (const char*)A);
                if (o0 + 8 > lim || o1 + 8 > lim) {
                    atomicAdd(&ctg_stem_oob<AR>[0], 1ull);
                    r[2 * q] = r[2 * q + 1] = c64{0.f, 0.f};
                    return;
                }
            }
#endif
            if (VEC) {
                const f32x4 v = *(const f32x4*)(sb + a_lane);
                r[2 * q] = c64{v[0], v[1]};
                r[2 * q + 1] = c64{v[2], v[3]};
            } else {
                const char* sb1 = (const char*)(A + (base + kj[2 * q + 1]));
                const float2 v0 = *(const float2*)(sb + a_lane);
                const float2 v1 = *(const float2*)(sb1 + a_lane);
                r[2 * q] = c64{v0.x, v0.y};
                r[2 * q + 1] = c64{v1.x, v1.y};
            }
        }
    };
    auto issue = [&](c64 (&r)[8], auto always_tag) __attribute__((always_inline)) {
        prep(always_tag);
        const int64_t base = pend0 + pend1 + pend2 + pend3;
#pragma unroll
        for (int q = 0; q < 4; ++q) fire2(r, q, base, always_tag);
    };

#ifdef CTG_STEM_TIMELINE
    int tl_n = 0;
#endif
    f32x16 ax[RT1], ay[RT1];
    f32x16 axm[XM1 ? RT1 : 1];
    constexpr int NST = PACK2 ? 8 : 16;
    float2 pv[RI2 ? 1 : NST];
    float* pdst = C;
    constexpr int NSET = RI2 ? (IT2 > 1 ? 2 : 1) : 1;
    f32x16 cr[NSET][2];
    auto store2 = [&](float* q, float2 v) __attribute__((always_inline)) {
#ifdef CTG_STEM_BOUNDS
        if ((uint64_t)((char*)q - (char*)C) + 8 > (uint64_t)p.c_elems * 8) {
            atomicAdd(&ctg_stem_oob<AR>[1], 1ull);
            return;
        }
#endif
        if constexpr (STEM_NT_STORES) {
            typedef float f32x2 __attribute__((ext_vector_type(2)));
            __builtin_nontemporal_store(f32x2{v.x, v.y}, (f32x2*)q);
        } else {
            *(float2*)q = v;
        }
    };
    auto drain = [&](int lo, int hi, auto set_tag, auto scaled_tag) __attribute__((always_inline)) {
        constexpr int SET = decltype(set_tag)::value < NSET ? decltype(set_tag)::value : 0;
#pragma unroll
        for (int i = lo; i < hi; ++i) {
            if constexpr (RI2) {
                float2 v;
                v.x = cr[SET][i >> 3][2 * (i & 7)];
                v.y = cr[SET][i >> 3][2 * (i & 7) + 1];
                if constexpr (decltype(scaled_tag)::value) {
                    v.x = v.x * alpha * alpha2;
                    v.y = v.y * alpha * alpha2;
                }
                store2(pdst + 2 * out_t(i), v);
            } else {
                store2(pdst + 2 * out_t(PACK2 ? 2 * i : i), pv[i]);
            }
        }
    };
    auto consume = [&](c64 (&r)[8], int m, int ch, auto always_tag, auto drain_tag, auto scaled_tag)
                       __attribute__((always_inline)) {
        constexpr bool DRAIN = decltype(drain_tag)::value >= 0;
        const int64_t base = pend0 + pend1 + pend2 + pend3;
        if constexpr (BF3) {
            float re[8], im[8];
#pragma unroll
            for (int j = 0; j < 8; ++j) {
                re[j] = r[j].re;
                im[j] = r[j].im;
            }
            bf16x8 r3[3], i3[3], n3[3], bp3[CG1][3], bq3[CG1][3];
            AR::split(re, r3, h2_sa);
            AR::split(im, i3, h2_sa);
            __builtin_amdgcn_sched_barrier(0);
            constexpr bool GP = STEM_GATHER_PORTIONS && decltype(always_tag)::value;
            if constexpr (!GP) {
#pragma unroll
                for (int q = 0; q < 4; ++q) fire2(r, q, base, always_tag);
            }
#pragma unroll
            for (int q = 0; q < 3; ++q) {
                if (!PACK1 && !XM1) n3[q] = __builtin_bit_cast(bf16x8, __builtin_bit_cast(u32x4, i3[q]) ^ 0x80008000u);
#pragma unroll
                for (int cg = 0; cg < CG1; ++cg) {
                    if constexpr (BR1) {
                        bp3[cg][q] = b1r3[cg][ch][q][0];
                        bq3[cg][q] = b1r3[cg][ch][q][1];
                    } else {
                        bp3[cg][q] = *(const bf16x8*)(q1p + cg * q1cg + ch * 48 + q * 8);
                        bq3[cg][q] = *(const bf16x8*)(q1q + cg * q1cg + ch * 48 + q * 8);
                    }
                }
            }
            __builtin_amdgcn_sched_barrier(0);
            const bool fresh = XM && STATIC && ch == 0;
            f32x16 zero16;
#pragma unroll
            for (int u = 0; u < 16; ++u) zero16[u] = 0.f;
#pragma unroll
            for (int t = 0; t < 6; t += AR::t_step(t)) {
                const int ta = bf3_ta(t), tb = bf3_tb(t);
                if constexpr (GP) {
                    constexpr int P = AR::products;
                    const int i = AR::t_index(t);
#pragma unroll
                    for (int q = (4 * i + P - 1) / P; q < (4 * (i + 1) + P - 1) / P; ++q) fire2(r, q, base, always_tag);
                }
                if (PACK1) {
                    ax[m] = AR::mfma(r3[ta], bp3[0][tb], (fresh && t == 0) ? zero16 : ax[m]);
                    ax[m] = AR::mfma(i3[ta], bq3[0][tb], ax[m]);
                } else if constexpr (XM1) {
                    ax[m] = AR::mfma(r3[ta], bp3[0][tb], (fresh && t == 0) ? zero16 : ax[m]);
                    ay[m] = AR::mfma(r3[ta], bq3[0][tb], (fresh && t == 0) ? zero16 : ay[m]);
                    axm[m] = AR::mfma(i3[ta], bq3[0][tb], (fresh && t == 0) ? zero16 : axm[m]);
                    ay[m] = AR::mfma(i3[ta], bp3[0][tb], ay[m]);
                } else {
#pragma unroll
                    for (int cg = 0; cg < CG1; ++cg) {
                        const int u = m * CG1 + cg;
                        ax[u] = AR::mfma(r3[ta], bp3[cg][tb], (fresh && t == 0) ? zero16 : ax[u]);
                        ay[u] = AR::mfma(r3[ta], bq3[cg][tb], (fresh && t == 0) ? zero16 : ay[u]);
                    }
#pragma unroll
                    for (int cg = 0; cg < CG1; ++cg) {
                        const int u = m * CG1 + cg;
                        ax[u] = AR::mfma(n3[ta], bq3[cg][tb], ax[u]);
                        ay[u] = AR::mfma(i3[ta], bp3[cg][tb], ay[u]);
                    }
                }
// ... 57 lines not shown
            for (int t = 0; t < 16; ++t) {
                dst[mid_t(t)] = XM1 ? ax[m][t] - axm[m][t] : ax[m][t];
                if constexpr (RI2) {
                    if constexpr (PACK1) {
                        if (l31 >> 4) dst[LD2 + mid_t(t)] = -ax[m][t];
                    } else {
                        dst[LD2 + mid_t(t)] = ay[m][t];
                        dst[2 * LD2 + mid_t(t)] = -ay[m][t];
                    }
                } else {
                    if (!PACK1) dst[PLANE1 + mid_t(t)] = ay[m][t];
                }
            }
        }
    };
    auto item_row = [&](int item, int64_t c_tile) __attribute__((always_inline)) -> int64_t {
        const int cg = item / n_rt2, rt2 = item - cg * n_rt2;
        int64_t c_row = c_tile + sload64(p.out_row + 32 * rt2);
        asm volatile("" : "+s"(c_row));
        return c_row;
    };
    auto item2r = [&](int rt2, int64_t c_row, auto set_tag, auto prev_tag, auto scaled_tag) __attribute__((always_inline)) {
        constexpr int SET = decltype(set_tag)::value;
        constexpr bool DRAIN = decltype(prev_tag)::value >= 0;
        const float* a0p = mid + ri_plane + (rt2 * 32 + (l31 >> 1)) * RP;
        const float* a1p = a0p + 16 * RP;
        const int64_t c_col = oc_s[ri_cg * 32 + l31];
        f32x4 a0[2], a1[2], bq[2];
        a0[0] = *(const f32x4*)(a0p);
        a1[0] = *(const f32x4*)(a1p);
        constexpr int NQ = K2Q > 0 ? K2Q : 1;
        if constexpr (K2Q > 0) {
            static_for<0, NQ>([&](auto qi) __attribute__((always_inline)) {
                constexpr int q = decltype(qi)::value;
                if (q + 1 < NQ) {
                    a0[(q + 1) & 1] = *(const f32x4*)(a0p + (q + 1) * 4);
                    a1[(q + 1) & 1] = *(const f32x4*)(a1p + (q + 1) * 4);
                }
                __builtin_amdgcn_sched_barrier(0);
#pragma unroll
                for (int t = 0; t < 4; ++t) {
                    if (q == 0 && t == 0) {
                        f32x16 z;
#pragma unroll
                        for (int u = 0; u < 16; ++u) z[u] = 0.f;
                        cr[SET][0] = mfma(a0[0][0], b2r[0][0][0], z);
                        cr[SET][1] = mfma(a1[0][0], b2r[0][0][0], z);
                    } else {
                        cr[SET][0] = mfma(a0[q & 1][t], b2r[q][0][t], cr[SET][0]);
                        cr[SET][1] = mfma(a1[q & 1][t], b2r[q][0][t], cr[SET][1]);
                    }
                }
                __builtin_amdgcn_sched_barrier(0);
                if constexpr (DRAIN) drain(q * NST / NQ, (q + 1) * NST / NQ, prev_tag, scaled_tag);
            });
        } else {
            if constexpr (DRAIN) drain(0, NST, prev_tag, scaled_tag);
#pragma unroll
            for (int u = 0; u < 16; ++u) cr[SET][0][u] = cr[SET][1][u] = 0.f;
            const int nq = K2 >> 2;
            bq[0] = *(const f32x4*)(ri_b);
            for (int kq = 0; kq < nq; kq += 2) {
#pragma unroll
                for (int h = 0; h < 2; ++h) {
                    const int nx = (kq + h + 1 < nq ? kq + h + 1 : nq - 1) * 4;
                    a0[(h + 1) & 1] = *(const f32x4*)(a0p + nx);
                    a1[(h + 1) & 1] = *(const f32x4*)(a1p + nx);
                    bq[(h + 1) & 1] = *(const f32x4*)(ri_b + nx);
                    __builtin_amdgcn_sched_barrier(0);
#pragma unroll
                    for (int t = 0; t < 4; ++t) {
                        cr[SET][0] = mfma(a0[h][t], bq[h][t], cr[SET][0]);
                        cr[SET][1] = mfma(a1[h][t], bq[h][t], cr[SET][1]);
                    }
                    __builtin_amdgcn_sched_barrier(0);
                }
            }
        }
        pdst = C + 2 * (c_row + out_lane + c_col);
    };
    auto item2 = [&](int item, int64_t c_row, auto scaled_tag, auto drain_tag, auto defer_tag)
                     __attribute__((always_inline)) {
        constexpr bool DRAIN = decltype(drain_tag)::value;
        if constexpr (DRAIN && (K2Q == 0 || BF3)) drain(0, NST, std::integral_constant<int, 0>{}, scaled_tag);
        const int cg = item / n_rt2, rt2 = item - cg * n_rt2;
        f32x16 cx, cy;
        if constexpr (!XM2) {
#pragma unroll
            for (int t = 0; t < 16; ++t) {
                cx[t] = 0.f;
                if (!PACK2) cy[t] = 0.f;
            }
        }
        const float* a_base = mid + kk * PLANE + (rt2 * 32 + l31) * LD2;
        const float* bxp = b2x + cg * 32 * LDB2;
        const float* byp = PACK2 ? nullptr : b2y + cg * 32 * LDB2;
        const int64_t c_col = oc_s[PACK2 ? (l31 & 15) : cg * 32 + l31];
        const int nq = K2 >> 2;
        f32x4 af[2], bx[2], by[2];
        f32x16 cxm;
        if constexpr (XM2) {
            const unsigned short* bR = Q2 + (cg * 32 + l31) * ROW2 + kk * 24;
            const unsigned short* bI = bR + N2 * ROW2;
            const float* aRf = mid + (rt2 * 32 + l31) * LD2 + kk * 8;
            struct Frag { bf16x8 ar[3], ai[3], br[3], bi[3]; };
            auto load_frag = [&](Frag& F, int c) __attribute__((always_inline)) {
                const f32x4 r0 = *(const f32x4*)(aRf + 16 * c), r1 = *(const f32x4*)(aRf + 16 * c + 4);
                const f32x4 i0 = *(const f32x4*)(aRf + PLANE + 16 * c), i1 = *(const f32x4*)(aRf + PLANE + 16 * c + 4);
                const float re8[8] = {r0[0], r0[1], r0[2], r0[3], r1[0], r1[1], r1[2], r1[3]};
                const float im8[8] = {i0[0], i0[1], i0[2], i0[3], i1[0], i1[1], i1[2], i1[3]};
                AR::split(re8, F.ar, h2_st);
                AR::split(im8, F.ai, h2_st);
#pragma unroll
                for (int q = 0; q < 3; ++q) {
                    F.br[q] = *(const bf16x8*)(bR + c * 48 + q * 8);
                    F.bi[q] = *(const bf16x8*)(bI + c * 48 + q * 8);
                }
            };
            auto mul_frag = [&](const Frag& F, auto first_tag) __attribute__((always_inline)) {
                constexpr bool FIRST = decltype(first_tag)::value;
                f32x16 zero16;
#pragma unroll
                for (int u = 0; u < 16; ++u) zero16[u] = 0.f;
#pragma unroll
                for (int t = 0; t < 6; t += AR::t_step(t)) {
                    const int ta = bf3_ta(t), tb = bf3_tb(t);
                    cx = AR::mfma(F.ar[ta], F.br[tb], (FIRST && t == 0) ? zero16 : cx);
                    cy = AR::mfma(F.ar[ta], F.bi[tb], (FIRST && t == 0) ? zero16 : cy);
                    cxm = AR::mfma(F.ai[ta], F.bi[tb], (FIRST && t == 0) ? zero16 : cxm);
                    cy = AR::mfma(F.ai[ta], F.br[tb], cy);
                }
            };
            const int nc = K2 >> 4;
            if constexpr (WS) {
                Frag F0, F1;
                load_frag(F0, 0);
                if (nc == 1) {
                    mul_frag(F0, std::true_type{});
                } else {
                    load_frag(F1, 1);
                    mul_frag(F0, std::true_type{});
                    for (int c = 2; c < nc; c += 2) {
                        load_frag(F0, c);
                        mul_frag(F1, std::false_type{});
                        load_frag(F1, c + 1);
                        mul_frag(F0, std::false_type{});
                    }
                    mul_frag(F1, std::false_type{});
                }
            } else {
                Frag F0;
                load_frag(F0, 0);
                mul_frag(F0, std::true_type{});
                for (int c = 1; c < nc; ++c) {
                    load_frag(F0, c);
                    mul_frag(F0, std::false_type{});
                }
            }
        } else if constexpr (BF3) {
            const unsigned short* bxq = q2x + (PACK2 ? 0 : cg * 32 * ROW2);
            const unsigned short* byq = PACK2 ? nullptr : q2y + cg * 32 * ROW2;
            for (int kb = 0; kb < (K2 >> 3); ++kb) {
                const f32x4 lo = *(const f32x4*)(a_base + 8 * kb), hi = *(const f32x4*)(a_base + 8 * kb + 4);
                const float a8[8] = {lo[0], lo[1], lo[2], lo[3], hi[0], hi[1], hi[2], hi[3]};
                bf16x8 a3[3], ax3[3], bx3[3], by3[3];
                AR::split(a8, a3, h2_st);
#pragma unroll
                for (int q = 0; q < 3; ++q) {
                    ax3[q] = PACK2 ? a3[q]
                                   : __builtin_bit_cast(bf16x8, __builtin_bit_cast(u32x4, a3[q]) ^ (sgn2 | (sgn2 >> 16)));
                    bx3[q] = *(const bf16x8*)(bxq + kb * 24 + q * 8);
                    if (!PACK2) by3[q] = *(const bf16x8*)(byq + kb * 24 + q * 8);
                }
#pragma unroll
                for (int t = 0; t < 6; t += AR::t_step(t)) {
                    cx = AR::mfma(ax3[bf3_ta(t)], bx3[bf3_tb(t)], cx);
                    if (!PACK2) cy = AR::mfma(a3[bf3_ta(t)], by3[bf3_tb(t)], cy);
                }
            }
        } else {
        af[0] = *(const f32x4*)(a_base);
        if constexpr (K2Q > 0) {
#pragma unroll
            for (int kq = 0; kq < K2Q; ++kq) {
                if (kq + 1 < K2Q) af[(kq + 1) & 1] = *(const f32x4*)(a_base + (kq + 1) * 4);
                __builtin_amdgcn_sched_barrier(0);
#pragma unroll
                for (int t = 0; t < 4; ++t) {
                    if (PACK2) {
                        cx = mfma(af[kq & 1][t], b2r[kq][0][t], cx);
                    } else {
                        cx = mfma(af[kq & 1][t], b2r[kq][0][t], cx);
                        cy = mfma(af[kq & 1][t], b2r[kq][PACK2 ? 0 : 1][t], cy);
                    }
                }
                __builtin_amdgcn_sched_barrier(0);
                if constexpr (DRAIN && !BF3) drain(kq * NST / K2Q, (kq + 1) * NST / K2Q, std::integral_constant<int, 0>{}, scaled_tag);
            }
        } else {
        bx[0] = *(const f32x4*)(bxp);
        if (!PACK2) by[0] = *(const f32x4*)(byp);
        for (int kq = 0; kq < nq; kq += 2) {
#pragma unroll
            for (int h = 0; h < 2; ++h) {
                const int nx = (kq + h + 1 < nq ? kq + h + 1 : nq - 1) * 4;
                af[(h + 1) & 1] = *(const f32x4*)(a_base + nx);
                bx[(h + 1) & 1] = *(const f32x4*)(bxp + nx);
                if (!PACK2) by[(h + 1) & 1] = *(const f32x4*)(byp + nx);
                __builtin_amdgcn_sched_barrier(0);
#pragma unroll
                for (int t = 0; t < 4; ++t) {
                    if (PACK2) {
                        cx = mfma(af[h][t], bx[h][t], cx);
                    } else {
                        cx = mfma(flip(af[h][t], sgn2), bx[h][t], cx);
                        cy = mfma(af[h][t], by[h][t], cy);
                    }
                }
                __builtin_amdgcn_sched_barrier(0);
            }
        }
        }
        }
        {
            constexpr bool SC = decltype(scaled_tag)::value;
            pdst = C + 2 * (c_row + out_lane + c_col);
            if (PACK2) {
                const bool hi = (l31 >> 4) != 0;
#pragma unroll
                for (int t = 0; t < 16; t += 2) {
                    const float mine = hi ? cx[t] : cx[t + 1];
                    const float got = __builtin_bit_cast(
                        float, __builtin_amdgcn_ds_swizzle(__builtin_bit_cast(int, mine), 0x401F));
                    float2 v;
                    v.x = hi ? got : cx[t];
                    v.y = hi ? cx[t + 1] : got;
                    if (SC) {
                        v.x = v.x * alpha * alpha2;
                        v.y = v.y * alpha * alpha2;
                    }
                    if constexpr (BF3) h2_vmax = fmaxf(h2_vmax, fmaxf(fabsf(v.x), fabsf(v.y)));
                    pv[t >> 1] = v;
                }
            } else {
#pragma unroll
                for (int t = 0; t < 16; ++t) {
                    float2 v;
                    const float xr = XM2 ? cx[t] - cxm[t] : cx[t];
                    v.x = SC ? xr * alpha * alpha2 : xr;
                    v.y = SC ? cy[t] * alpha * alpha2 : cy[t];
                    if constexpr (BF3) h2_vmax = fmaxf(h2_vmax, fmaxf(fabsf(v.x), fabsf(v.y)));
                    pv[t] = v;
                }
            }
            if constexpr (!decltype(defer_tag)::value) drain(0, NST, std::integral_constant<int, 0>{}, scaled_tag);
        }
    };
    auto item2k = [&](auto nc_tag, int item0, int64_t c_row, auto scaled_tag) __attribute__((always_inline)) {
        constexpr int NC = decltype(nc_tag)::value;
        constexpr bool SC = decltype(scaled_tag)::value;
        const int cg0 = item0 / n_rt2, rt2 = item0 - cg0 * n_rt2;
        const int cgs = PW / n_rt2;
        const int bI = N2 * ROW2;
        const float* aRf = mid + (rt2 * 32 + l31) * LD2 + kk * 8;
        struct FragA { bf16x8 ar[3], ai[3]; };
        struct FragB { bf16x8 br[3], bi[3]; };
        FragA AK[NC];
        FragB BF[2];
        f32x16 cx, cy, cxm;
        auto load_a = [&](FragA& F, int c) __attribute__((always_inline)) {
            const f32x4 r0 = *(const f32x4*)(aRf + 16 * c), r1 = *(const f32x4*)(aRf + 16 * c + 4);
            const f32x4 i0 = *(const f32x4*)(aRf + PLANE + 16 * c), i1 = *(const f32x4*)(aRf + PLANE + 16 * c + 4);
            const float re8[8] = {r0[0], r0[1], r0[2], r0[3], r1[0], r1[1], r1[2], r1[3]};
            const float im8[8] = {i0[0], i0[1], i0[2], i0[3], i1[0], i1[1], i1[2], i1[3]};
            AR::split(re8, F.ar, h2_st);
            AR::split(im8, F.ai, h2_st);
        };
        auto load_b = [&](FragB& F, const unsigned short* bR, int c) __attribute__((always_inline)) {
#pragma unroll
            for (int q = 0; q < 3; ++q) {
                F.br[q] = *(const bf16x8*)(bR + c * 48 + q * 8);
                F.bi[q] = *(const bf16x8*)(bR + bI + c * 48 + q * 8);
            }
        };
        auto mul = [&](const FragA& A_, const FragB& B_, bool first) __attribute__((always_inline)) {
            f32x16 zero16;
#pragma unroll
            for (int u = 0; u < 16; ++u) zero16[u] = 0.f;
#pragma unroll
            for (int t = 0; t < 6; t += AR::t_step(t)) {
                const int ta = bf3_ta(t), tb = bf3_tb(t);
                cx = AR::mfma(A_.ar[ta], B_.br[tb], (first && t == 0) ? zero16 : cx);
                cy = AR::mfma(A_.ar[ta], B_.bi[tb], (first && t == 0) ? zero16 : cy);
                cxm = AR::mfma(A_.ai[ta], B_.bi[tb], (first && t == 0) ? zero16 : cxm);
                cy = AR::mfma(A_.ai[ta], B_.br[tb], cy);
            }
        };
        auto emit = [&](int cg) __attribute__((always_inline)) {
            pdst = C + 2 * (c_row + out_lane + oc_s[cg * 32 + l31]);
#pragma unroll
            for (int t = 0; t < 16; ++t) {
                float2 v;
                const float xr = cx[t] - cxm[t];
                v.x = SC ? xr * alpha * alpha2 : xr;
                v.y = SC ? cy[t] * alpha * alpha2 : cy[t];
                h2_vmax = fmaxf(h2_vmax, fmaxf(fabsf(v.x), fabsf(v.y)));
                pv[t] = v;
            }
        };
        static_for<0, 2>([&](auto gi) __attribute__((always_inline)) {
            constexpr int G = decltype(gi)::value;
            const int cg = cg0 + G * cgs;
            const unsigned short* bR = Q2 + (cg * 32 + l31) * ROW2 + kk * 24;
            if constexpr (G == 1) drain(0, NST, std::integral_constant<int, 0>{}, scaled_tag);
            if constexpr (G == 0) load_a(AK[0], 0);
            load_b(BF[0], bR, 0);
            static_for<0, NC>([&](auto ci) __attribute__((always_inline)) {
                constexpr int CH = decltype(ci)::value;
                if constexpr (CH + 1 < NC) {
                    if constexpr (G == 0) load_a(AK[CH + 1], CH + 1);
                    load_b(BF[(CH + 1) & 1], bR, CH + 1);
                }
                mul(AK[CH], BF[CH & 1], CH == 0);
            });
            emit(cg);
        });
    };
    f32x16 mx[TRI ? ITM : 1], my[TRI ? ITM : 1];
    auto item_mid = [&](auto ii) __attribute__((always_inline)) {
        constexpr int I = decltype(ii)::value;
        f32x16 cx, cy;
#pragma unroll
        for (int t = 0; t < 16; ++t) {
            cx[t] = 0.f;
            cy[t] = 0.f;
        }
        const float* a_base = mid + kk * PLANEM + am_row[I];
        if constexpr (BF3) {
            for (int kb = 0; kb < (KM >> 3); ++kb) {
                const f32x4 lo = *(const f32x4*)(a_base + 8 * kb), hi = *(const f32x4*)(a_base + 8 * kb + 4);
                const float a8[8] = {lo[0], lo[1], lo[2], lo[3], hi[0], hi[1], hi[2], hi[3]};
                bf16x8 a3[3], ax3[3], bx3[3], by3[3];
                AR::split(a8, a3);
#pragma unroll
                for (int q = 0; q < 3; ++q) {
                    ax3[q] = PACKM ? a3[q]
                                   : __builtin_bit_cast(bf16x8, __builtin_bit_cast(u32x4, a3[q]) ^ (sgn2 | (sgn2 >> 16)));
                    bx3[q] = *(const bf16x8*)(qmx[I] + kb * 24 + q * 8);
                    if (!PACKM) by3[q] = *(const bf16x8*)(qmy[I] + kb * 24 + q * 8);
                }
#pragma unroll
                for (int t = 0; t < 6; t += AR::t_step(t)) {
                    cx = AR::mfma(ax3[bf3_ta(t)], bx3[bf3_tb(t)], cx);
                    if (!PACKM) cy = AR::mfma(a3[bf3_ta(t)], by3[bf3_tb(t)], cy);
                }
            }
        } else {
            const int nq = KM >> 2;
            f32x4 af[2], bx[2], by[2];
            af[0] = *(const f32x4*)(a_base);
            bx[0] = *(const f32x4*)(bmx[I]);
            if (!PACKM) by[0] = *(const f32x4*)(bmy[I]);
            for (int kq = 0; kq < nq; kq += 2) {
#pragma unroll
                for (int h = 0; h < 2; ++h) {
                    const int nx = (kq + h + 1 < nq ? kq + h + 1 : nq - 1) * 4;
                    af[(h + 1) & 1] = *(const f32x4*)(a_base + nx);
                    bx[(h + 1) & 1] = *(const f32x4*)(bmx[I] + nx);
                    if (!PACKM) by[(h + 1) & 1] = *(const f32x4*)(bmy[I] + nx);
                    __builtin_amdgcn_sched_barrier(0);
#pragma unroll
                    for (int t = 0; t < 4; ++t) {
                        if (PACKM) {
                            cx = mfma(af[h][t], bx[h][t], cx);
                        } else {
                            cx = mfma(flip(af[h][t], sgn2), bx[h][t], cx);
                            cy = mfma(af[h][t], by[h][t], cy);
                        }
                    }
                    __builtin_amdgcn_sched_barrier(0);
                }
            }
        }
        mx[I] = cx;
        my[I] = cy;
    };
    auto scatter_mid = [&](auto ii) __attribute__((always_inline)) {
        constexpr int I = decltype(ii)::value;
        float* dst = mid + (m2_lane[I] + m2_rt[I]);
#pragma unroll
        for (int t = 0; t < 16; ++t) {
            dst[m2_t(t)] = mx[I][t];
            if (!PACKM) dst[PLANE + m2_t(t)] = my[I][t];
        }
    };
    auto emit_one = [&](int m, int64_t c_tile, auto scaled_tag) __attribute__((always_inline)) {
        constexpr bool SC = decltype(scaled_tag)::value;
#pragma unroll
        for (int t = 0; t < 16; ++t) {
            float2 v;
            const float xr = XM1 ? ax[m][t] - axm[m][t] : ax[m][t];
            v.x = SC ? xr * alpha * alpha2 : xr;
            v.y = SC ? ay[m][t] * alpha * alpha2 : ay[m][t];
            if constexpr (BF3) h2_vmax = fmaxf(h2_vmax, fmaxf(fabsf(v.x), fabsf(v.y)));
            pv[RI2 ? 0 : t] = v;
        }
        pdst = C + 2 * (c_tile + one_rt[m] + out_lane + one_col);
    };
    int h2_par = 0;
    auto h2_publish = [&]() __attribute__((always_inline)) {
        if constexpr (AR::fp16 && !ONE) {
            float mx = 0.f;
#pragma unroll
            for (int m = 0; m < RT1; ++m)
#pragma unroll
                for (int t = 0; t < 16; ++t) {
                    const float xr = XM1 ? ax[m][t] - axm[m][t] : ax[m][t];
                    mx = fmaxf(mx, fabsf(xr));
                    if (!PACK1) mx = fmaxf(mx, fabsf(ay[m][t]));
                }
#pragma unroll
            for (int o = 32; o > 0; o >>= 1) mx = fmaxf(mx, __shfl_xor(mx, o));
            if (lane == 0) bf3_red[h2_par * 8 + wave1] = mx;
            if constexpr (WS) h2_par ^= 1;
        }
    };
    auto h2_consume = [&]() __attribute__((always_inline)) {
        if constexpr (AR::fp16 && !ONE) {
            float mx = bf3_red[h2_par * 8];
#pragma unroll
            for (int w = 1; w < PW; ++w) mx = fmaxf(mx, bf3_red[h2_par * 8 + w]);
            const int et = __builtin_amdgcn_readfirstlane(h2_exponent_of(mx));
            h2_st = pow2f(-et);
            h2_set_alpha(et);
            h2_par ^= 1;
        }
    };
    auto tile_c = [&](int64_t g) __attribute__((always_inline)) -> int64_t {
        const int64_t gh = g >> p.g_lo_shift, gl = g & (p.g_lo - 1);
        return sload64(p.gC_hi + uniform64(gh)) + sload64(p.gC_lo + uniform64(gl));
    };

    auto run = [&](auto scaled_tag) __attribute__((always_inline)) {
    if constexpr (WS) {
        constexpr int NT = RR1 * NCH;
        constexpr int U = (NT % GD == 0) ? 1 : ((2 * NT) % GD == 0 ? 2 : 4);
        static_assert((U * NT) % GD == 0, "a pass of U tiles returns to gather set 0");
        auto step1 = [&](auto slot0_tag) __attribute__((always_inline)) {
            constexpr int SLOT0 = decltype(slot0_tag)::value;
            static_for<0, RR1>([&](auto mi) __attribute__((always_inline)) {
                constexpr int M = decltype(mi)::value;
                static_for<0, NCH>([&](auto ci) __attribute__((always_inline)) {
                    constexpr int CH = decltype(ci)::value;
                    consume(regs[(SLOT0 + M * NCH + CH) & (GD - 1)], M, CH, std::true_type{}, std::integral_constant<int, -1>{}, scaled_tag);
                });
            });
        };
        auto step2 = [&](int64_t gc) __attribute__((always_inline)) {
            const int64_t c_tile = tile_c(gc);
            int64_t c_rows[IT2];
            if constexpr (IT2 == 2 && XM2) {
                if (n_rt2 <= PW) {
                    const int nc = K2 >> 4;
                    if (nc == 4) {
                        item2k(std::integral_constant<int, 4>{}, wave1, item_row(wave1, c_tile), scaled_tag);
                        return;
                    }
                    if (nc == 2) {
                        item2k(std::integral_constant<int, 2>{}, wave1, item_row(wave1, c_tile), scaled_tag);
                        return;
                    }
                }
            }
            static_for<0, IT2>([&](auto ii) __attribute__((always_inline)) {
                c_rows[decltype(ii)::value] = item_row(wave1 + PW * decltype(ii)::value, c_tile);
            });
            static_for<0, IT2>([&](auto ii) __attribute__((always_inline)) {
                constexpr int I = decltype(ii)::value;
                item2(wave1 + PW * I, c_rows[I], scaled_tag, std::integral_constant<bool, (I > 0)>{}, std::true_type{});
            });
        };
        if (producer) {
            static_for<0, GD>([&](auto gi) __attribute__((always_inline)) { issue(regs[decltype(gi)::value], std::true_type{}); });
            prep(std::true_type{});
            step1(std::integral_constant<int, 0>{});
            for (int64_t t = 0; t < my_tiles; t += U) {
                static_for<0, U>([&](auto ui) __attribute__((always_inline)) {
                    constexpr int UI = decltype(ui)::value;
                    if (t + UI < my_tiles) {
                        h2_publish();
                        __syncthreads();
                        scatter();
                        __syncthreads();
                        if (t + UI + 1 < my_tiles) step1(std::integral_constant<int, ((UI + 1) * NT) & (GD - 1)>{});
                    }
                });
            }
        } else {
            for (int64_t t = 0; t < my_tiles; ++t) {
                __syncthreads();
                if (t > 0) drain(0, NST, std::integral_constant<int, 0>{}, scaled_tag);
                __syncthreads();
                h2_consume();
                step2(tile0 + t * tile_step);
            }
            drain(0, NST, std::integral_constant<int, 0>{}, scaled_tag);
        }
    } else if constexpr (STATIC) {
        constexpr int NT = RT1 * NCH;
        constexpr int U = (NT % GD) ? 2 : 1;
        static_assert((U * NT) % GD == 0, "a pass of U tiles returns to gather set 0");
        constexpr int LASTSET = RI2 ? ((IT2 > 0 ? IT2 - 1 : 0) & (NSET - 1)) : 0;
        static_for<0, GD>([&](auto gi) __attribute__((always_inline)) { issue(regs[decltype(gi)::value], std::true_type{}); });
        prep(std::true_type{});
        int64_t g = tile0;
        auto tile = [&](auto slot0_tag, auto first_tag) __attribute__((always_inline)) {
            constexpr int SLOT0 = decltype(slot0_tag)::value;
            constexpr bool FIRST = decltype(first_tag)::value;
            if constexpr (ONE) {
                const int64_t c_tile = tile_c(g);
                static_for<0, RT1>([&](auto mi) __attribute__((always_inline)) {
                    constexpr int M = decltype(mi)::value;
                    zero_acc(M);
                    static_for<0, NCH>([&](auto ci) __attribute__((always_inline)) {
                        constexpr int CH = decltype(ci)::value;
                        consume(regs[(SLOT0 + M * NCH + CH) & (GD - 1)], M, CH, std::true_type{},
                                std::integral_constant<int, (CH == 0 && !(FIRST && M == 0)) ? 0 : -1>{}, scaled_tag);
                    });
                    emit_one(M, c_tile, scaled_tag);
                });
                g += tile_step;
                return;
            }
            CTG_TL_STAMP(0);
            static_for<0, RT1>([&](auto mi) __attribute__((always_inline)) {
                constexpr int M = decltype(mi)::value;
                zero_acc(M);
                static_for<0, NCH>([&](auto ci) __attribute__((always_inline)) {
                    constexpr int CH = decltype(ci)::value;
                    consume(regs[(SLOT0 + M * NCH + CH) & (GD - 1)], M, CH, std::true_type{},
                            std::integral_constant<int, (!FIRST && M == 0 && CH == 0) ? LASTSET : -1>{}, scaled_tag);
                });
            });
            CTG_TL_STAMP(1);
            h2_publish();
            __syncthreads();
            CTG_TL_STAMP(2);
// ... 24 lines not shown
                constexpr int I = decltype(ii)::value;
                if constexpr (RI2)
                    item2r(ri_rt0 + ri_rts * I, c_rows[I], std::integral_constant<int, I & (NSET - 1)>{},
                           std::integral_constant<int, (I > 0) ? ((I - 1) & (NSET - 1)) : -1>{}, scaled_tag);
                else
                    item2(wave + SW * I, c_rows[I], scaled_tag, std::integral_constant<bool, (I > 0)>{}, std::true_type{});
            });
            CTG_TL_STAMP(5);
            g += tile_step;
        };
        auto pass = [&](auto peel_tag) __attribute__((always_inline)) {
            static_for<0, U>([&](auto ui) __attribute__((always_inline)) {
                tile(std::integral_constant<int, (decltype(ui)::value * NT) & (GD - 1)>{},
                     std::integral_constant<bool, decltype(peel_tag)::value && decltype(ui)::value == 0>{});
            });
        };
        int64_t t = 0;
        if (my_tiles >= U) {
            pass(std::true_type{});
            for (t = U; t + U <= my_tiles; t += U) pass(std::false_type{});
        }
        if (t < my_tiles) {
            if (t == 0) tile(std::integral_constant<int, 0>{}, std::true_type{});
            else tile(std::integral_constant<int, 0>{}, std::false_type{});
        }
        drain(0, NST, std::integral_constant<int, LASTSET>{}, scaled_tag);
    } else {
        issue(regs[0], std::false_type{});
        issue(regs[1], std::false_type{});
        prep(std::false_type{});
        int slot = 0;
        for (int64_t g = tile0; g < n_tiles; g += tile_step) {
            const int64_t c_tile1 = ONE ? tile_c(g) : 0;
#pragma unroll
            for (int m = 0; m < RT1; ++m) {
                zero_acc(m);
                for (int ch = 0; ch < nch; ++ch) {
                    if (slot == 0) consume(regs[0], m, ch, std::false_type{}, std::integral_constant<int, -1>{}, scaled_tag);
                    else consume(regs[1], m, ch, std::false_type{}, std::integral_constant<int, -1>{}, scaled_tag);
                    slot ^= 1;
                }
                if constexpr (ONE) {
                    emit_one(m, c_tile1, scaled_tag);
                    drain(0, NST, std::integral_constant<int, 0>{}, scaled_tag);
                }
            }
            if constexpr (ONE) continue;
            h2_publish();
            __syncthreads();
            scatter();
            __syncthreads();
            h2_consume();
            const int64_t c_tile = tile_c(g);
            for (int item = wave; item < n_items; item += SW)
                item2(item, item_row(item, c_tile), scaled_tag, std::false_type{}, std::false_type{});
        }
    }
    };
    if (scaled) run(std::true_type{});
    else run(std::false_type{});
    if constexpr (BF3) {
        if (p.cmax != nullptr) {
            float mx = h2_vmax;
#pragma unroll
            for (int o = 32; o > 0; o >>= 1) mx = fmaxf(mx, __shfl_xor(mx, o));
            if (lane == 0 && mx > 0.f && mx < __builtin_bit_cast(float, 0x7f800000u))
                record_max(p.cmax, mx);
        }
    }
}

template <bool PACK1, bool PACK2, int RT1_, int CS1, int NCH, int IT2_, bool BR1 = false, int K2Q = 0, bool VEC = false,
          bool BF3 = false, bool RI2 = false, bool ONE = false, int ITM = 0, bool PACKM = false, bool XM = false,
          bool LM = false, bool WS = false>
__global__ __launch_bounds__(SW * 64, 1) void stem2_kernel(StemArgs p) {
    stem2_body<Bf16x3, PACK1, PACK2, RT1_, CS1, NCH, IT2_, BR1, K2Q, VEC, BF3, RI2, ONE, ITM, PACKM, XM, LM, WS>(p);
}
template <bool PACK1, bool PACK2, int RT1_, int CS1, int NCH, int IT2_, bool BR1 = false, int K2Q = 0, bool VEC = false,
          bool BF3 = false, bool RI2 = false, bool ONE = false, int ITM = 0, bool PACKM = false, bool XM = false,
          bool LM = false, bool WS = false>
__global__ __launch_bounds__(SW * 64, 1) void stem2h_kernel(StemArgs p) {
    stem2_body<Fp16x2, PACK1, PACK2, RT1_, CS1, NCH, IT2_, BR1, K2Q, VEC, BF3, RI2, ONE, ITM, PACKM, XM, LM, WS>(p);
}

#ifdef CTG_STEM_TIMELINE
template <class AR>
int stem_debug_timeline(unsigned long long* out, int reset) {
    if (hipDeviceSynchronize() != hipSuccess) return -1;
    if (hipMemcpyFromSymbol(out, HIP_SYMBOL(ctg_stem_tl<AR>), sizeof(unsigned long long) * 8 * CTG_TL_TILES * 6) != hipSuccess) return -1;
    if (reset) {
        static unsigned long long z[8 * CTG_TL_TILES * 6];
        if (hipMemcpyToSymbol(HIP_SYMBOL(ctg_stem_tl<AR>), z, sizeof(z)) != hipSuccess) return -1;
    }
    return 0;
}
#endif

#ifdef CTG_STEM_BOUNDS
template <class AR>
int stem_debug_oob(unsigned long long out[2], int reset) {
    if (hipMemcpyFromSymbol(out, HIP_SYMBOL(ctg_stem_oob<AR>), 16) != hipSuccess) return -1;
    if (reset) {
        const unsigned long long z[2] = {0, 0};
        if (hipMemcpyToSymbol(HIP_SYMBOL(ctg_stem_oob<AR>), z, 16) != hipSuccess) return -1;
    }
    return 0;
}
#endif

#ifndef CTG_STEM_DEV_ONE
template <class AR, auto... A>
static auto stem_kernel() {
    if constexpr (AR::fp16) return stem2h_kernel<A...>;
    else return stem2_kernel<A...>;
}

static size_t stem2_lds_bytes(const StemArgs& p) {
    const size_t b1 = (size_t)(p.N1 == 16 ? 3 : 2) * p.N1 * (p.K1 + 4);
    const size_t b2 = (size_t)(p.N2 == 16 ? 3 : 2) * p.N2 * (p.K2 + 4);
    const size_t mid = (size_t)2 * p.rows2 * p.ld2;
    return 4 * (b1 + b2 + mid) + 8 * (size_t)p.N2;
}

static size_t stem2_lds_bytes_bf3(const StemArgs& p) {
    const size_t q1 = (size_t)(p.N1 == 16 ? 3 : 2) * p.N1 * ((p.K1 >> 4) * 48 + 8);
    const size_t q2 = (size_t)(p.N2 == 16 ? 3 : 2) * p.N2 * ((p.K2 >> 3) * 24 + 8);
    return 2 * (q1 + q2) + 4 * (size_t)2 * p.rows2 * p.ld2 + 8 * (size_t)p.N2 + 64;
}

static size_t stem2_lds_bytes_ri2(const StemArgs& p, bool b2_in_regs) {
    const size_t b1 = (size_t)(p.N1 == 16 ? 3 : 2) * p.N1 * (p.K1 + 4);
    const size_t b2 = (size_t)2 * p.N2 * (p.K2 + 4);
    const size_t mid = (size_t)3 * p.rows2 * p.ld2;
    return 4 * (b1 + (b2_in_regs ? (mid > b2 ? mid : b2) : b2 + mid)) + 8 * (size_t)p.N2;
}

template <class AR, bool PACK1, bool PACK2, int RT1, int CS1, int NCH, int IT2, bool BR1 = false, int K2Q = 0, bool VEC = false,
          bool BF3 = false, bool RI2 = false, bool XM = false, bool WS = false>
static hipError_t launch_stem2_t(const StemArgs& p, hipStream_t stream) {
    auto kern = stem_kernel<AR, PACK1, PACK2, RT1, CS1, NCH, IT2, BR1, K2Q, VEC, BF3, RI2, false, 0, false, XM, false, WS>();
    static unsigned long long ready = 0;
    {
        const hipError_t e = lds_opt_in((const void*)kern, 160 * 1024, &ready);
        if (e != hipSuccess) return e;
    }
#ifdef CTG_STEM_TIMELINE
    {
        static int taken = 0;
        int on = 0, k1 = 0, n1 = 0, k2 = 0, n2 = 0;
        if (const char* v = getenv("CTG_TL_SHAPE"))
            if (sscanf(v, "%d,%d,%d,%d", &k1, &n1, &k2, &n2) == 4 && k1 == p.K1 && n1 == p.N1 && k2 == p.K2 && n2 == p.N2 && !taken)
                on = taken = 1;
        (void)hipMemcpyToSymbolAsync(HIP_SYMBOL(ctg_stem_tl_on<AR>), &on, sizeof(int), 0, hipMemcpyHostToDevice, stream);
    }
#endif
    const size_t smem = BF3 ? stem2_lds_bytes_bf3(p) : (RI2 ? stem2_lds_bytes_ri2(p, K2Q > 0) : stem2_lds_bytes(p));
    int64_t blocks = p.n_tiles < 256 ? p.n_tiles : 256;
    hipLaunchKernelGGL(kern, dim3((unsigned)blocks, 1), dim3(SW * 64), smem, stream, p);
    return hipGetLastError();
}

static size_t stem2_lds_bytes_one(const StemArgs& p, bool bf3) {
    if (bf3) return 2 * (size_t)2 * p.N1 * ((p.K1 >> 4) * 48 + 8) + 8 * (size_t)p.N1 + 64;
    return 4 * (size_t)2 * p.N1 * (p.K1 + 4) + 8 * (size_t)p.N1;
}

template <class AR, int RT1, int CS1, int NCH, bool BR1, bool VEC, bool BF3>
static hipError_t launch_stem1_t(const StemArgs& p, hipStream_t stream) {
    constexpr bool XM = BF3 && NCH > 0;
    auto kern = stem_kernel<AR, false, false, RT1, CS1, NCH, 0, BR1, 0, VEC, BF3, false, true, 0, false, XM, false, false>();
    static unsigned long long ready = 0;
    {
        const hipError_t e = lds_opt_in((const void*)kern, 160 * 1024, &ready);
        if (e != hipSuccess) return e;
    }
    int64_t blocks = p.n_tiles < 256 ? p.n_tiles : 256;
    hipLaunchKernelGGL(kern, dim3((unsigned)blocks, 1), dim3(SW * 64), stem2_lds_bytes_one(p, BF3), stream, p);
    return hipGetLastError();
}

static size_t stem3_lds_bytes(const StemArgs& p, bool bf3) {
    const size_t m1 = (size_t)p.rowsM * p.ldM, m2 = (size_t)p.rows2 * p.ld2;
    const size_t mid = 8 * (m1 > m2 ? m1 : m2);
    auto planes = [](int n) { return (size_t)(n == 16 ? 3 : 2); };
    if (bf3) {
        const size_t q = planes(p.N1) * p.N1 * ((p.K1 >> 4) * 48 + 8) + planes(p.NM) * p.NM * ((p.KM >> 3) * 24 + 8) +
                         planes(p.N2) * p.N2 * ((p.K2 >> 3) * 24 + 8);
        return 2 * q + mid + 8 * (size_t)p.N2 + 64;
    }
    const size_t b = planes(p.N1) * p.N1 * (p.K1 + 4) + planes(p.NM) * p.NM * (p.KM + 4) + planes(p.N2) * p.N2 * (p.K2 + 4);
    return 4 * b + mid + 8 * (size_t)p.N2;
}

template <bool P1, bool PM, bool P2, int RT1, int CS1, int NCH, int ITM, int IT2, bool VEC, bool BF3>
static hipError_t launch_stem3_t(const StemArgs& p, hipStream_t stream) {
    auto kern = stem2_kernel<P1, P2, RT1, CS1, NCH, IT2, (NCH <= 2), 0, VEC, BF3, false, false, ITM, PM>;
    static unsigned long long ready = 0;
    {
        const hipError_t e = lds_opt_in((const void*)kern, 160 * 1024, &ready);
        if (e != hipSuccess) return e;
    }
    int64_t blocks = p.n_tiles < 256 ? p.n_tiles : 256;
    hipLaunchKernelGGL(kern, dim3((unsigned)blocks, 1), dim3(SW * 64), stem3_lds_bytes(p, BF3), stream, p);
    return hipGetLastError();
}

#if !defined(CTG_STEM_TRIPLES_BUILD)
#define CTG_STEM_TRI(X)
#elif defined(CTG_STEM_TRI_DEV)
#define CTG_STEM_TRI(X) \
    X(true, true, true, 2, 1, 1, 2, 2, false) X(false, false, false, 1, 1, 2, 1, 1, false) \
    X(true, false, true, 2, 1, 1, 1, 1, false) X(true, false, false, 1, 1, 1, 1, 1, true)
#else
#define CTG_STEM_TRI(X) \
    X(true, true, false, 2, 1, 1, 2, 1, true) X(true, true, false, 2, 1, 1, 2, 1, false) \
    X(true, false, true, 2, 1, 1, 1, 2, false) X(false, true, true, 1, 1, 2, 2, 2, false) \
    X(false, true, false, 1, 2, 1, 2, 2, false) X(false, false, true, 1, 1, 2, 1, 2, false) \
    X(false, false, true, 1, 1, 4, 1, 1, true) \
    X(true, false, true, 2, 1, 1, 1, 1, false) X(true, false, true, 2, 1, 1, 1, 1, true) \
    X(false, true, true, 1, 4, 2, 2, 2, true) X(false, false, false, 1, 1, 2, 1, 4, false) \
    X(true, false, false, 1, 1, 1, 1, 1, true)
#endif

static bool stem3_instantiated(bool p1, bool pm, bool p2, int rt1, int cs1, int nch, int itm, int it2, bool vec) {
#define CTG_STEM_HAS3(A, M, B, R, CS, NC, IM, IT, V) \
    if (p1 == A && pm == M && p2 == B && rt1 == R && cs1 == CS && nch == NC && itm == IM && it2 == IT && vec == V) return true;
// ... 347 lines not shown
```

### cotengra_amd/runtime.py

```python

from __future__ import annotations

import ctypes as C
import os

import numpy as np

_LIB_PATH = os.environ.get("CTG_LIB") or os.path.join(os.path.dirname(os.path.abspath(__file__)), "lib", "libctg_hip.so")
ABI_VERSION = 10

SYMBOLS = (
    "ctg_abi_version",
    "ctg_last_error",
    "ctg_plan_create",
    "ctg_plan_destroy",
    "ctg_plan_nslices",
    "ctg_plan_workspace_bytes",
    "ctg_exec_create",
    "ctg_exec_destroy",
    "ctg_exec_set_stream",
    "ctg_exec_upload_inputs_host",
    "ctg_exec_upload_inputs_device",
    "ctg_exec_zero_result",
    "ctg_exec_set_strip_exponent",
    "ctg_exec_set_stem_arithmetic",
    "ctg_exec_get_exponent",
    "ctg_exec_run_slices",
    "ctg_exec_run_slice_list",
    "ctg_plan_share_units",
    "ctg_plan_share_slice_ids",
    "ctg_exec_run_share",
    "ctg_exec_slice_batch",
    "ctg_exec_device_bytes",
    "ctg_stem_triple_instantiated",
    "ctg_exec_launch_count",
    "ctg_exec_profile_slice",
    "ctg_exec_step_kernel",
    "ctg_exec_sync",
    "ctg_exec_result_ptr",
    "ctg_exec_result_stats",
    "ctg_exec_sample_result",
    "ctg_exec_sample_info",
    "ctg_exec_range_audit",
    "ctg_exec_result_topk",
    "ctg_exec_result_marginal",
    "ctg_exec_result_rdm",
    "ctg_exec_download_result",
    "ctg_exec_download_arena",
    "ctg_exec_get_state",
    "ctg_exec_set_state",
    "ctg_exec_state_dtype",
    "ctg_exec_get_state_wide",
    "ctg_exec_set_state_wide",
    "ctg_comm_get_unique_id",
    "ctg_comm_init",
    "ctg_comm_info",
    "ctg_comm_destroy",
    "ctg_exec_reduce",
    "ctg_path_greedy",
    "ctg_slice_greedy",
    "ctg_subtree_reconfigure",
    "ctg_subtree_reconfigure_timed",
)


class CtgError(RuntimeError):
    """A call into libctg_hip.so failed."""


class CommError(CtgError):
    """RCCL is missing or a collective failed (CTG_E_COMM)."""


class PlanDesc(C.Structure):

    _fields_ = [
        ("dtype", C.c_int32),
        ("n_inputs", C.c_int64),
        ("input_sizes", C.POINTER(C.c_int64)),
        ("input_offsets", C.POINTER(C.c_int64)),
        ("inputs_elems", C.c_int64),
        ("arena_elems", C.c_int64),
        ("result_elems", C.c_int64),
        ("n_steps", C.c_int64),
        ("steps", C.POINTER(C.c_int64)),
        ("n_table_words", C.c_int64),
        ("tables", C.POINTER(C.c_int64)),
        ("n_sliced", C.c_int64),
        ("slice_sizes", C.POINTER(C.c_int64)),
        ("slice_fixed", C.POINTER(C.c_int64)),
        ("slice_strides", C.POINTER(C.c_int64)),
        ("slice_group", C.POINTER(C.c_int64)),
    ]


_lib = None


def lib_path():
    return _LIB_PATH


def load():
    global _lib
    if _lib is not None:
        return _lib
    if not os.path.exists(_LIB_PATH):
        raise ImportError(
            f"{_LIB_PATH} not found: build the HIP extension first "
            "(python -c 'import __graft_entry__ as g; g.build()'). "
            "cotengra_amd has no CPU fallback."
        )
    try:
        import torch
    except ImportError:
        pass
    lib = C.CDLL(_LIB_PATH)
    i64p = C.POINTER(C.c_int64)
    vp = C.c_void_p
    lib.ctg_abi_version.restype = C.c_int
    lib.ctg_last_error.restype = C.c_char_p
    protos = {
        "ctg_plan_create": [C.POINTER(PlanDesc), C.POINTER(vp)],
        "ctg_plan_destroy": [vp],
        "ctg_plan_nslices": [vp, i64p],
        "ctg_plan_workspace_bytes": [vp, i64p],
        "ctg_exec_create": [vp, C.c_int, vp, vp, C.POINTER(vp)],
        "ctg_exec_destroy": [vp],
        "ctg_exec_set_stream": [vp, vp],
        "ctg_exec_upload_inputs_host": [vp, C.POINTER(vp)],
        "ctg_exec_upload_inputs_device": [vp, C.POINTER(vp)],
        "ctg_exec_zero_result": [vp],
        "ctg_exec_set_strip_exponent": [vp, C.c_int, C.c_int],
        "ctg_exec_set_stem_arithmetic": [vp, C.c_int],
        "ctg_exec_get_exponent": [vp, C.POINTER(C.c_double), C.POINTER(C.c_int)],
        "ctg_exec_run_slices": [vp, C.c_int64, C.c_int64, C.c_int64],
        "ctg_exec_run_slice_list": [vp, i64p, C.c_int64],
        "ctg_plan_share_units": [vp, C.c_int64, C.c_int64, i64p, i64p],
        "ctg_plan_share_slice_ids": [vp, C.c_int64, C.c_int64, C.c_int64, C.c_int64, i64p],
        "ctg_exec_run_share": [vp, C.c_int64, C.c_int64, C.c_int64, C.c_int64],
        "ctg_exec_slice_batch": [vp, i64p],
        "ctg_exec_device_bytes": [vp, i64p],
        "ctg_stem_triple_instantiated": [C.c_int] * 9,
        "ctg_exec_launch_count": [vp, i64p, i64p],
        "ctg_exec_profile_slice": [vp, C.c_int64, C.POINTER(C.c_float)],
        "ctg_exec_step_kernel": [vp, C.c_int64, C.c_char_p, C.c_int64],
        "ctg_exec_sync": [vp],
        "ctg_exec_result_ptr": [vp, C.POINTER(vp)],
        "ctg_exec_result_stats": [vp, C.POINTER(C.c_double), C.POINTER(C.c_double), C.POINTER(C.c_double), i64p],
        "ctg_exec_sample_result": [vp, C.POINTER(C.c_double), C.c_int64, i64p, vp, C.POINTER(C.c_double)],
        "ctg_exec_sample_info": [vp, C.POINTER(C.c_double), C.POINTER(C.c_double), C.POINTER(C.c_double), i64p,
                                 C.POINTER(C.c_float)],
        "ctg_exec_range_audit": [vp, C.c_int64, i64p, C.POINTER(C.c_double)],
        "ctg_exec_result_topk": [vp, C.c_int64, i64p, vp, C.POINTER(C.c_double)],
        "ctg_exec_result_marginal": [vp, C.c_int64, i64p, C.POINTER(C.c_int32), C.POINTER(C.c_double)],
        "ctg_exec_result_rdm": [vp, C.c_int64, i64p, C.POINTER(C.c_int32), vp],
        "ctg_exec_download_result": [vp, vp],
        "ctg_exec_download_arena": [vp, C.c_int64, C.c_int64, vp],
        "ctg_exec_get_state": [vp, vp, C.POINTER(C.c_double), C.POINTER(C.c_int)],
        "ctg_exec_set_state": [vp, vp, C.c_double, C.c_int],
        "ctg_exec_state_dtype": [vp, C.POINTER(C.c_int)],
        "ctg_exec_get_state_wide": [vp, vp, C.POINTER(C.c_double), C.POINTER(C.c_int)],
        "ctg_exec_set_state_wide": [vp, vp, C.c_double, C.c_int],
        "ctg_comm_get_unique_id": [vp],
        "ctg_comm_init": [vp, C.c_int, C.c_int, C.c_int, C.POINTER(vp)],
        "ctg_comm_info": [vp, C.POINTER(C.c_int), C.POINTER(C.c_int), C.POINTER(C.c_int)],
        "ctg_comm_destroy": [vp],
        "ctg_exec_reduce": [vp, vp, C.c_int],
        "ctg_path_greedy": [C.c_int64, i64p, i64p, C.c_int64, i64p, C.c_int64, C.POINTER(C.c_double),
                            C.c_double, C.c_double, C.c_int64, C.c_uint64, i64p],
        "ctg_slice_greedy": [C.c_int64, i64p, i64p, C.c_int64, i64p, C.c_int64, C.POINTER(C.c_double),
                             i64p, C.c_double, C.c_int, C.c_int64, i64p, i64p],
        "ctg_subtree_reconfigure": [C.c_int64, i64p, i64p, C.c_int64, i64p, C.c_int64, C.POINTER(C.c_double),
                                    i64p, C.c_int64, C.c_int64, C.c_double, i64p],
        "ctg_subtree_reconfigure_timed": [C.c_int64, i64p, i64p, C.c_int64, i64p, C.c_int64,
                                          C.POINTER(C.c_double), i64p, C.c_int64, C.c_int64,
                                          C.POINTER(C.c_double), C.c_int64, C.c_double, i64p],
    }
    for name, argtypes in protos.items():
        fn = getattr(lib, name)
        fn.argtypes = argtypes
        fn.restype = C.c_int
    if lib.ctg_abi_version() != ABI_VERSION:
        raise ImportError(
            f"libctg_hip.so ABI {lib.ctg_abi_version()} != expected {ABI_VERSION}; rebuild."
        )
    _lib = lib
    return lib


def _check(rc):
    if rc != 0:
        msg = load().ctg_last_error().decode("utf-8", "replace")
        if rc in (-1, -6):
            raise ValueError(msg)
        if rc == -3:
            raise MemoryError(msg)
        if rc == -5:
            raise CommError(msg)
        raise CtgError(f"[{rc}] {msg}")


def _i64p(arr):
    return arr.ctypes.data_as(C.POINTER(C.c_int64))


def check_topk_k(k):
    import operator

    if isinstance(k, (bool, np.bool_)):
        raise TypeError(f"k = {k!r} is not an integer.")
    try:
        k = operator.index(k)
    except TypeError:
        raise TypeError(f"k = {k!r} is not an integer.") from None
    if k < 1:
        raise ValueError(f"k = {k}: need at least 1.")
    return k


def rdm_dim(extents, keep):
    d = 1
    for n, f in zip(extents, keep):
        if n < 1:
            raise ValueError(f"extent {n} is not positive.")
        if f == 1:
            d *= int(n)
    if d > Executor.RDM_MAX_DIM:
        raise ValueError(f"rdm: the kept extents' product is {d}; at most {Executor.RDM_MAX_DIM} (CTG_RDM_MAX_DIM).")
    return d


def rdm_variant(dtype, extents, keep):
    t = {"float32": "float", "float64": "double", "complex64": "c64", "complex128": "c128"}[np.dtype(dtype).name]
    ext = [int(n) for n in extents]
    d = rdm_dim(ext, list(keep))
    n = 1
    for v in ext:
        n *= v
    if n >= 4096 and all(v & (v - 1) == 0 for v in ext):
        return f"rdm_chunk_kernel<{t},{max(d, 16) // 16}>"
    return f"rdm_general_kernel<{t}>"


class DevicePlan:

    def __init__(self, plan):
        self.plan = plan
        lib = load()
        s = plan.serialise()
        self._keep = s
        d = PlanDesc()
        d.dtype = s["dtype"]
        d.n_inputs = len(s["input_sizes"])
        d.input_sizes = _i64p(s["input_sizes"])
        d.input_offsets = _i64p(s["input_offsets"])
        d.inputs_elems = plan.inputs_elems
        d.arena_elems = s["arena_elems"]
        d.result_elems = s["result_elems"]
        d.n_steps = s["n_steps"]
        d.steps = _i64p(s["steps"])
        d.n_table_words = len(s["tables"])
        d.tables = _i64p(s["tables"])
        d.n_sliced = len(s["slice_sizes"])
        d.slice_sizes = _i64p(s["slice_sizes"])
        d.slice_fixed = _i64p(s["slice_fixed"])
        d.slice_strides = _i64p(s["slice_strides"])
        d.slice_group = _i64p(s["slice_group"])
        handle = C.c_void_p()
        _check(lib.ctg_plan_create(C.byref(d), C.byref(handle)))
        self.handle = handle
        self._keep = None

    @property
    def nslices(self):
        n = C.c_int64()
        _check(load().ctg_plan_nslices(self.handle, C.byref(n)))
        return n.value

    def share_units(self, rank=0, world=1):
        u, g = C.c_int64(), C.c_int64()
        _check(load().ctg_plan_share_units(self.handle, int(rank), int(world), C.byref(u), C.byref(g)))
        return u.value, g.value

    def share_slice_ids(self, rank=0, world=1, unit_first=0, unit_count=-1):
        units, gsize = self.share_units(rank, world)
        n = units - unit_first if unit_count < 0 else unit_count
        out = np.empty(max(n, 0) * gsize, dtype=np.int64)
        _check(load().ctg_plan_share_slice_ids(self.handle, int(rank), int(world), int(unit_first), int(n), _i64p(out)))
        return out

    def workspace_bytes(self):
        out = (C.c_int64 * 4)()
        _check(load().ctg_plan_workspace_bytes(self.handle, out))
        return dict(zip(("inputs", "arena", "result", "tables"), out))

    def close(self):
        if getattr(self, "handle", None):
            load().ctg_plan_destroy(self.handle)
            self.handle = None

    def __del__(self):
        try:
            self.close()
        except Exception:
            pass


class Executor:

    def __init__(self, dplan, device=0, stream=0, result_ptr=None):
        self.dplan = dplan
        self.plan = dplan.plan
        self.device = int(device)
        handle = C.c_void_p()
        _check(
            load().ctg_exec_create(
                dplan.handle,
                self.device,
                C.c_void_p(int(stream) if stream else None),
                C.c_void_p(int(result_ptr) if result_ptr else None),
                C.byref(handle),
            )
        )
        self.handle = handle

    def set_stream(self, stream):
        _check(load().ctg_exec_set_stream(self.handle, C.c_void_p(int(stream) if stream else None)))


    def upload_host(self, arrays):
        dt = np.dtype(self.plan.dtype)
        keep = [np.ascontiguousarray(x, dtype=dt) for x in arrays]
        self._check_sizes([x.size for x in keep])
        ptrs = (C.c_void_p * len(keep))(*[x.ctypes.data for x in keep])
        _check(load().ctg_exec_upload_inputs_host(self.handle, ptrs))

    def upload_device(self, ptrs, sizes):
        self._check_sizes(sizes)
        arr = (C.c_void_p * len(ptrs))(*[int(p) for p in ptrs])
        _check(load().ctg_exec_upload_inputs_device(self.handle, arr))

    def _check_sizes(self, sizes):
        want = list(self.plan.input_sizes)
        if list(sizes) != want:
            raise ValueError(
                f"Input sizes {list(sizes)} do not match the plan's {want}."
            )


    def zero_result(self):
        _check(load().ctg_exec_zero_result(self.handle))

    def set_strip_exponent(self, strip, check_zero=False):
        _check(load().ctg_exec_set_strip_exponent(self.handle, int(bool(strip)), int(bool(check_zero))))

    STEM_ARITHMETICS = {"fp32": 0, "bf16x3": 1, "fp16x2": 2}

    def set_stem_arithmetic(self, mode):
        if mode is True:
            mode = 1
        elif mode is False:
            mode = 0
        elif isinstance(mode, str):
            mode = self.STEM_ARITHMETICS[mode]
        _check(load().ctg_exec_set_stem_arithmetic(self.handle, int(mode)))

    def get_exponent(self):
        e, z = C.c_double(), C.c_int()
        _check(load().ctg_exec_get_exponent(self.handle, C.byref(e), C.byref(z)))
        return e.value, bool(z.value)

    def run_slice_list(self, ids):
        arr = np.ascontiguousarray(ids, dtype=np.int64)
        _check(load().ctg_exec_run_slice_list(self.handle, arr.ctypes.data_as(C.POINTER(C.c_int64)), arr.size))

    def run_share(self, rank=0, world=1, unit_first=0, unit_count=-1):
        _check(load().ctg_exec_run_share(self.handle, int(rank), int(world), int(unit_first), int(unit_count)))

    def run_slices(self, first=0, count=None, stride=1):
        if count is None:
            count = (self.plan.nslices - first + stride - 1) // stride
        _check(load().ctg_exec_run_slices(self.handle, first, count, stride))

    @property
    def batch(self):
        n = C.c_int64()
        _check(load().ctg_exec_slice_batch(self.handle, C.byref(n)))
        return n.value

    def device_bytes(self):
        n = C.c_int64()
        _check(load().ctg_exec_device_bytes(self.handle, C.byref(n)))
        return n.value

    def launch_count(self):
        ns, nl = C.c_int64(), C.c_int64()
        _check(load().ctg_exec_launch_count(self.handle, C.byref(ns), C.byref(nl)))
        return ns.value, nl.value

    def profile_slice(self, slice_id=0):
        ms = (C.c_float * max(len(self.plan.steps), 1))()
        _check(load().ctg_exec_profile_slice(self.handle, slice_id, ms))
        return np.asarray(ms[: len(self.plan.steps)], dtype=np.float64)

    def step_kernels(self):
        buf = C.create_string_buffer(160)
        names = []
        for s in range(len(self.plan.steps)):
            _check(load().ctg_exec_step_kernel(self.handle, s, buf, 160))
            names.append(buf.value.decode())
        return names

    def sync(self):
        _check(load().ctg_exec_sync(self.handle))

    def result_ptr(self):
        p = C.c_void_p()
        _check(load().ctg_exec_result_ptr(self.handle, C.byref(p)))
        return p.value

    def download_result(self):
        out = np.empty(self.plan.result_shape, dtype=np.dtype(self.plan.dtype))
        _check(load().ctg_exec_download_result(self.handle, C.c_void_p(out.ctypes.data)))
        return out


    def result_stats(self):
        s, q, m, i = C.c_double(), C.c_double(), C.c_double(), C.c_int64()
        _check(load().ctg_exec_result_stats(self.handle, C.byref(s), C.byref(q), C.byref(m), C.byref(i)))
        return s.value, q.value, m.value, i.value

    def sample_result(self, uniforms):
        u = np.ascontiguousarray(uniforms, dtype=np.float64).reshape(-1)
        n = u.size
        idx = np.empty(n, dtype=np.int64)
        elems = np.empty(n, dtype=np.dtype(self.plan.dtype))
        p = np.empty(n, dtype=np.float64)
        dp = C.POINTER(C.c_double)
        _check(load().ctg_exec_sample_result(self.handle, u.ctypes.data_as(dp), n, _i64p(idx),
                                             C.c_void_p(elems.ctypes.data), p.ctypes.data_as(dp)))
        return idx, elems, p

    def sample_info(self):
        s, q, m, i = C.c_double(), C.c_double(), C.c_double(), C.c_int64()
        ms = (C.c_float * 2)()
        _check(load().ctg_exec_sample_info(self.handle, C.byref(s), C.byref(q), C.byref(m), C.byref(i), ms))
        return s.value, q.value, m.value, i.value, (ms[0], ms[1])


    TOPK_MAX = 1 << 20

    def topk_result(self, k):
        k = check_topk_k(k)
        idx = np.empty(k, dtype=np.int64)
        elems = np.empty(k, dtype=np.dtype(self.plan.dtype))
        p = np.empty(k, dtype=np.float64)
        _check(load().ctg_exec_result_topk(self.handle, k, _i64p(idx), C.c_void_p(elems.ctypes.data),
                                           p.ctypes.data_as(C.POINTER(C.c_double))))
        return idx, elems, p

    def marginal_result(self, extents, keep):
        ext = np.ascontiguousarray(extents, dtype=np.int64).reshape(-1)
        kp = np.ascontiguousarray(keep, dtype=np.int32).reshape(-1)
        if ext.size != kp.size:
            raise ValueError(f"{ext.size} extents and {kp.size} keep entries.")
        m = 1
        for d, f in zip(ext.tolist(), kp.tolist()):
            if d < 1:
                raise ValueError(f"extent {d} is not positive.")
            if f == 1:
                m *= d
        out = np.empty(m, dtype=np.float64)
        _check(load().ctg_exec_result_marginal(self.handle, ext.size, _i64p(ext), kp.ctypes.data_as(C.POINTER(C.c_int32)),
                                               out.ctypes.data_as(C.POINTER(C.c_double))))
        return out


    RDM_MAX_DIM = 64

    def rdm_result(self, extents, keep):
        ext = np.ascontiguousarray(extents, dtype=np.int64).reshape(-1)
        kp = np.ascontiguousarray(keep, dtype=np.int32).reshape(-1)
        if ext.size != kp.size:
            raise ValueError(f"{ext.size} extents and {kp.size} keep entries.")
        d = rdm_dim(ext.tolist(), kp.tolist())
        cplx = np.dtype(self.plan.dtype).kind == "c"
        out = np.empty((d, d), dtype=np.complex128 if cplx else np.float64)
        _check(load().ctg_exec_result_rdm(self.handle, ext.size, _i64p(ext), kp.ctypes.data_as(C.POINTER(C.c_int32)),
                                          C.c_void_p(out.ctypes.data)))
        return out

    def rdm_variant(self, extents, keep):
        return rdm_variant(self.plan.dtype, extents, keep)


# ... 105 lines not shown
```

### include/ctg_hip.h

```cpp
#ifndef CTG_HIP_H
#define CTG_HIP_H

#include <stdint.h>

#ifdef __cplusplus
extern "C" {
#endif

#define CTG_ABI_VERSION 10

enum { CTG_F32 = 0, CTG_F64 = 1, CTG_C64 = 2, CTG_C128 = 3 };

enum {
    CTG_OK = 0,
    CTG_E_INVALID = -1,
    CTG_E_HIP = -2,
    CTG_E_NOMEM = -3,
    CTG_E_BOUNDS = -4,
    CTG_E_COMM = -5,
    CTG_E_NORM = -6
};

#define CTG_STEP_WORDS 48

typedef struct ctg_plan_desc {
    int32_t dtype;
    int64_t n_inputs;
    const int64_t* input_sizes;
    const int64_t* input_offsets;
    int64_t inputs_elems;
    int64_t arena_elems;
    int64_t result_elems;
    int64_t n_steps;
    const int64_t* steps;
    int64_t n_table_words;
    const int64_t* tables;
    int64_t n_sliced;
    const int64_t* slice_sizes;
    const int64_t* slice_fixed;
    const int64_t* slice_strides;
    const int64_t* slice_group;
} ctg_plan_desc;

typedef struct ctg_plan ctg_plan;
typedef struct ctg_exec ctg_exec;
typedef struct ctg_comm ctg_comm;

int ctg_abi_version(void);
const char* ctg_last_error(void);

int ctg_plan_create(const ctg_plan_desc* desc, ctg_plan** out);
int ctg_plan_destroy(ctg_plan* plan);
int ctg_plan_nslices(const ctg_plan* plan, int64_t* nslices);
int ctg_plan_workspace_bytes(const ctg_plan* plan, int64_t bytes[4]);

int ctg_exec_create(const ctg_plan* plan, int device, void* stream,
                    void* ext_result, ctg_exec** out);
int ctg_exec_destroy(ctg_exec* exec);
int ctg_exec_set_stream(ctg_exec* exec, void* stream);

int ctg_exec_upload_inputs_host(ctg_exec* exec, const void* const* ptrs);
int ctg_exec_upload_inputs_device(ctg_exec* exec, const void* const* ptrs);

int ctg_exec_zero_result(ctg_exec* exec);

int ctg_exec_set_strip_exponent(ctg_exec* exec, int strip_exponent, int check_zero);

int ctg_exec_set_stem_arithmetic(ctg_exec* exec, int mode);
int ctg_exec_get_exponent(ctg_exec* exec, double* exponent, int* zero);

int ctg_exec_run_slices(ctg_exec* exec, int64_t first, int64_t count, int64_t stride);

int ctg_exec_slice_batch(ctg_exec* exec, int64_t* batch);
int ctg_exec_run_slice_list(ctg_exec* exec, const int64_t* ids, int64_t n);
int ctg_plan_share_units(const ctg_plan* plan, int64_t rank, int64_t world, int64_t* units, int64_t* slices_per_unit);
int ctg_plan_share_slice_ids(const ctg_plan* plan, int64_t rank, int64_t world, int64_t unit_first,
                             int64_t unit_count, int64_t* ids);
int ctg_exec_run_share(ctg_exec* exec, int64_t rank, int64_t world, int64_t unit_first, int64_t unit_count);
int ctg_exec_device_bytes(ctg_exec* exec, int64_t* bytes);
int ctg_stem_triple_instantiated(int p1, int pm, int p2, int rt1, int cs1, int nch, int itm, int it2, int vec);

int ctg_exec_launch_count(ctg_exec* exec, int64_t* steps, int64_t* launches);

int ctg_exec_profile_slice(ctg_exec* exec, int64_t slice_id, float* ms);

int ctg_exec_step_kernel(ctg_exec* exec, int64_t step, char* buf, int64_t buflen);

int ctg_exec_sync(ctg_exec* exec);
int ctg_exec_result_ptr(ctg_exec* exec, void** dev_ptr);
int ctg_exec_download_result(ctg_exec* exec, void* host_out);
int ctg_exec_result_stats(ctg_exec* exec, double* sum_p, double* sum_p2, double* max_p, int64_t* argmax);
int ctg_exec_sample_result(ctg_exec* exec, const double* u, int64_t n, int64_t* idx, void* elems, double* p);
int ctg_exec_sample_info(ctg_exec* exec, double* sum_p, double* sum_p2, double* max_p, int64_t* argmax, float* pass_ms);
#define CTG_RANGE_WORDS 260
int ctg_exec_range_audit(ctg_exec* exec, int64_t slice_id, int64_t* rows, double* sumsq);
#define CTG_TOPK_MAX (1 << 20)
int ctg_exec_result_topk(ctg_exec* exec, int64_t k, int64_t* idx, void* elems, double* p);
#define CTG_MARGINAL_PARTIALS (1 << 22)
int ctg_exec_result_marginal(ctg_exec* exec, int64_t rank, const int64_t* extents, const int32_t* keep, double* out);
#define CTG_RDM_MAX_DIM 64
int ctg_exec_result_rdm(ctg_exec* exec, int64_t rank, const int64_t* extents, const int32_t* keep, void* out);
int ctg_exec_download_arena(ctg_exec* exec, int64_t offset, int64_t n, void* host_out);

int ctg_exec_get_state(ctg_exec* exec, void* host_result, double* exponent, int* zero);
int ctg_exec_set_state(ctg_exec* exec, const void* host_result, double exponent, int zero);
int ctg_exec_state_dtype(ctg_exec* exec, int* dtype);
int ctg_exec_get_state_wide(ctg_exec* exec, void* host_sum, double* exponent, int* zero);
int ctg_exec_set_state_wide(ctg_exec* exec, const void* host_sum, double exponent, int zero);

#define CTG_UNIQUE_ID_BYTES 128
int ctg_comm_get_unique_id(void* id_out );
int ctg_comm_init(const void* id, int rank, int world, int device, ctg_comm** out);
int ctg_comm_info(const ctg_comm* comm, int* rank, int* world, int* device);
int ctg_comm_destroy(ctg_comm* comm);
int ctg_exec_reduce(ctg_exec* exec, ctg_comm* comm, int root);


int ctg_path_greedy(int64_t n_inputs, const int64_t* offsets, const int64_t* inds, int64_t n_out,
                    const int64_t* out_inds, int64_t n_inds, const double* sizes, double costmod,
                    double temperature, int64_t max_neighbors, uint64_t seed, int64_t* ssa_path);

int ctg_slice_greedy(int64_t n_inputs, const int64_t* offsets, const int64_t* inds, int64_t n_out,
                     const int64_t* out_inds, int64_t n_inds, const double* sizes,
                     const int64_t* ssa_path, double target_log2_size, int allow_outer,
                     int64_t max_sliced, int64_t* sliced, int64_t* n_sliced);

int ctg_subtree_reconfigure(int64_t n_inputs, const int64_t* offsets, const int64_t* inds, int64_t n_out,
                            const int64_t* out_inds, int64_t n_inds, const double* sizes,
                            const int64_t* ssa_path_in, int64_t subtree_size, int64_t maxiter,
                            double write_factor, int64_t* ssa_path_out);

int ctg_subtree_reconfigure_timed(int64_t n_inputs, const int64_t* offsets, const int64_t* inds,
                                  int64_t n_out, const int64_t* out_inds, int64_t n_inds,
                                  const double* sizes, const int64_t* ssa_path_in, int64_t subtree_size,
                                  int64_t maxiter, const double* mac_rate_by_log2k, int64_t n_rates,
                                  double elem_rate, int64_t* ssa_path_out);

#ifdef __cplusplus
}
#endif
#endif
```

Measured before the change: 173000 billion FLOP/s.

## Pair adjacent output columns in stem kernels for 16-byte stores

Adds a paired-store variant of the stem pair kernels. Each wave's two items now cover adjacent even/odd output columns of the same row tile, so results are written as 16-byte vectors instead of two 8-byte float2 stores. A host-side plan check confirms the output column, row and offset tables are even-aligned and the C pointer is 16-byte aligned before enabling it. Item-to-column mapping changes and the variant only applies to specific shapes (fp16x2 WS with IT2=1 by default, symmetric path behind a compile flag). It also adds introspection APIs for paired-store status and the recorded stem maximum.

```diff
diff --git a/cotengra_amd/csrc/ctg_common.h b/cotengra_amd/csrc/ctg_common.h
--- a/cotengra_amd/csrc/ctg_common.h
+++ b/cotengra_amd/csrc/ctg_common.h
@@ -164,6 +164,7 @@
     int64_t a_elems, c_elems;
     const float* amax;
     float* cmax;
+    int32_t pair16;
 };
 
 __device__ __forceinline__ int64_t zid(const StepArgs& p) { return (int64_t)p.z0 + blockIdx.y; }
@@ -456,6 +457,8 @@
 bool stem2_uses_bf3(const StemArgs& p);
 hipError_t launch_stem2h(const StemArgs& p, hipStream_t stream);
 void stem2h_kernel_name(const StemArgs& p, char* buf, size_t n);
+int stem2_last_paired();
+int stem2h_last_paired();
 
 hipError_t launch_single(int dtype, const StepArgs& p, hipStream_t stream);
 bool pair_bf16x3_on(const StepArgs& p);
diff --git a/cotengra_amd/csrc/ctg_exec_state.h b/cotengra_amd/csrc/ctg_exec_state.h
--- a/cotengra_amd/csrc/ctg_exec_state.h
+++ b/cotengra_amd/csrc/ctg_exec_state.h
@@ -58,6 +58,7 @@
     int64_t plan_steps = 0;
     std::vector<char> rec_wanted;
     std::vector<char> wave_member;
+    std::vector<char> stem_paired_ran;
     std::vector<char> stem_h2_ran;
     std::vector<ctg::MfmaHints> hints;
     std::vector<ctg::MfmaHints> hints_b;
diff --git a/cotengra_amd/csrc/ctg_runtime.hip b/cotengra_amd/csrc/ctg_runtime.hip
--- a/cotengra_amd/csrc/ctg_runtime.hip
+++ b/cotengra_amd/csrc/ctg_runtime.hip
@@ -178,6 +178,28 @@
                         sl, op.name, (long long)hi, (long long)cap);
     }
     return CTG_OK;
+}
+
+bool stem_pair16_ok(const ctg_plan* p, int64_t s) {
+    const int64_t* r = &p->steps[s * STEP_WORDS];
+    const int64_t* h = &p->tables[r[W_STEM]];
+    if (h[SW_ONE] == 1 || h[SW_TRI] == 1) return false;
+    const int64_t N2 = h[SW_N2], rows2 = h[SW_ROWS2], n_tiles = h[SW_NTILES], g_lo = h[SW_GLO];
+    if (N2 < 2 || (N2 & 1)) return false;
+    const int64_t* oc = &p->tables[h[SW_TABS + ST_OUT_COL]];
+    for (int64_t j = 0; j < N2; j += 2)
+        if ((oc[j] & 1) || oc[j + 1] != oc[j] + 1) return false;
+    const int even_tabs[3] = {ST_OUT_ROW, ST_GC_HI, ST_GC_LO};
+    const int64_t len[3] = {rows2, n_tiles / g_lo, g_lo};
+    for (int t = 0; t < 3; ++t)
+        for (int64_t i = 0; i < len[t]; ++i)
+            if (p->tables[h[SW_TABS + even_tabs[t]] + i] & 1) return false;
+    if (r[W_C_OFF] & 1) return false;
+    if (r[W_C_SPACE] == SPACE_ARENA && (p->arena_elems & 1)) return false;
+    if (r[W_C_LEAF] >= 0)
+        for (int64_t j = 0; j < p->n_sliced; ++j)
+            if (p->slice_strides[r[W_C_LEAF] * p->n_sliced + j] & 1) return false;
+    return true;
 }
 
 int validate_plan(ctg_plan* p) {
@@ -508,6 +530,7 @@
             q.bf3 = e->stem_bf16x3;
             q.a_elems = r[W_A_SIZE];
             q.c_elems = r[W_C_SIZE];
+            q.pair16 = stem_pair16_ok(p, s) && ((uintptr_t)q.C & 15) == 0 ? 1 : 0;
             const int64_t** tabs[ST_COUNT] = {&q.gA_hi, &q.gA_lo, &q.gC_hi, &q.gC_lo, &q.kj_a, &q.lane_a, &q.rt_a,
                                               &q.chunk_a, &q.b1_off, &q.b2_off, &q.mid_row, &q.mid_col,
                                               &q.out_row, &q.out_col};
@@ -1128,6 +1151,7 @@
                     q.amax = slot;
                 }
                 if (err == hipSuccess) err = h2 ? launch_stem2h(q, stream) : launch_stem2(q, stream);
+                if (err == hipSuccess) e->stem_paired_ran[s] = (char)(h2 ? stem2h_last_paired() : stem2_last_paired());
             }
             break;
         }
@@ -1822,6 +1846,7 @@
                 }
             }
             e->stem_h2_ran.assign(p->n_steps, 0);
+            e->stem_paired_ran.assign(p->n_steps, 0);
             if (e->wave_member.size() != (size_t)p->n_steps) e->wave_member.assign(p->n_steps, 0);
             (void)stems;
             if (p->dtype == CTG_C64) {
@@ -2422,6 +2447,37 @@
     return CTG_OK;
 }
 
+int ctg_plan_stem_pair16(ctg_plan* p, int64_t step, int* ok) {
+    if (!p || !ok) return fail(CTG_E_INVALID, "null argument");
+    if (step < 0 || step >= p->n_steps) return fail(CTG_E_INVALID, "step out of range");
+    *ok = p->steps[step * STEP_WORDS + W_KIND] == KIND_STEM2 && stem_pair16_ok(p, step) ? 1 : 0;
+    return CTG_OK;
+}
+
+int ctg_exec_step_paired_stores(ctg_exec* e, int64_t step, int* paired) {
+    if (!e || !paired) return fail(CTG_E_INVALID, "null argument");
+    if (step < 0 || step >= e->plan->n_steps) return fail(CTG_E_INVALID, "step out of range");
+    *paired = (size_t)step < e->stem_paired_ran.size() && e->stem_paired_ran[step] ? 1 : 0;
+    return CTG_OK;
+}
+
+int ctg_exec_step_stem_max(ctg_exec* e, int64_t step, int64_t z, float* mx) {
+    if (!e || !mx) return fail(CTG_E_INVALID, "null argument");
+    const ctg_plan* p = e->plan;
+    if (step < 0 || step >= p->n_steps) return fail(CTG_E_INVALID, "step out of range");
+    if (z < 0 || z >= (e->batch > 1 ? e->batch : 1)) return fail(CTG_E_INVALID, "slice of the batch out of range");
+    if (e->d_stem_max == nullptr || (size_t)step >= e->stem_h2_ran.size() || !e->stem_h2_ran[step] ||
+        p->steps[step * STEP_WORDS + W_KIND] != KIND_STEM2)
+        return fail(CTG_E_INVALID, "step %lld has recorded no maximum", (long long)step);
+    HIP_TRY(hipSetDevice(e->device));
+    HIP_TRY(hipStreamSynchronize(e->stream));
+    float rec[kMaxSub];
+    HIP_TRY(hipMemcpy(rec, e->smax_slot(0, step, (e->invariant[step] || e->grouped[step]) ? 0 : z), sizeof(rec), hipMemcpyDeviceToHost));
+    *mx = rec[0];
+    for (int i = 1; i < kMaxSub; ++i) *mx = std::max(*mx, rec[i]);
+    return CTG_OK;
+}
+
 int ctg_exec_sync(ctg_exec* e) {
     if (!e) return fail(CTG_E_INVALID, "null argument");
     HIP_TRY(hipSetDevice(e->device));
diff --git a/cotengra_amd/csrc/ctg_stem.hip b/cotengra_amd/csrc/ctg_stem.hip
--- a/cotengra_amd/csrc/ctg_stem.hip
+++ b/cotengra_amd/csrc/ctg_stem.hip
@@ -2,8 +2,13 @@
 
 namespace ctg {
 #ifdef CTG_STEM_DEV_ONE
+#ifdef CTG_STEM_DEV_P16
+template __global__ void stem2_kernel_p16<CTG_STEM_DEV_ONE>(StemArgs);
+#else
 template __global__ void stem2_kernel<CTG_STEM_DEV_ONE>(StemArgs);
+#endif
 #else
+int stem2_last_paired() { return stem_last_paired; }
 bool stem2_supported(const StemArgs& p) { return stem2_supported_shape(p); }
 bool stem3_supported(const StemArgs& p) { return stem3_supported_shape(p); }
 bool stem2_uses_bf3(const StemArgs& p) { return stem_uses_16bit(p); }
diff --git a/cotengra_amd/csrc/ctg_stem_h2.hip b/cotengra_amd/csrc/ctg_stem_h2.hip
--- a/cotengra_amd/csrc/ctg_stem_h2.hip
+++ b/cotengra_amd/csrc/ctg_stem_h2.hip
@@ -2,8 +2,13 @@
 
 namespace ctg {
 #ifdef CTG_STEM_DEV_ONE
+#ifdef CTG_STEM_DEV_P16
+template __global__ void stem2h_kernel_p16<CTG_STEM_DEV_ONE>(StemArgs);
+#else
 template __global__ void stem2h_kernel<CTG_STEM_DEV_ONE>(StemArgs);
+#endif
 #else
+int stem2h_last_paired() { return stem_last_paired; }
 bool stem2h_supported(const StemArgs& p) { return stem2_supported_shape(p); }
 bool stem2h_uses_h2(const StemArgs& p) { return stem_uses_16bit(p); }
 void stem2h_kernel_name(const StemArgs& p, char* buf, size_t n) { stem_kernel_name<Fp16x2>(p, buf, n); }
diff --git a/cotengra_amd/csrc/ctg_stem_impl.h b/cotengra_amd/csrc/ctg_stem_impl.h
--- a/cotengra_amd/csrc/ctg_stem_impl.h
+++ b/cotengra_amd/csrc/ctg_stem_impl.h
@@ -241,9 +241,11 @@
 constexpr bool STEM_NT_STORES = CTG_STEM_NT_STORES != 0;
 constexpr bool STEM_GATHER_PORTIONS = CTG_STEM_GATHER_PORTIONS != 0;
 template <class AR, bool PACK1, bool PACK2, int RT1_, int CS1, int NCH, int IT2_, bool BR1, int K2Q, bool VEC, bool BF3,
-          bool RI2, bool ONE, int ITM, bool PACKM, bool XM, bool LM, bool WS>
+          bool RI2, bool ONE, int ITM, bool PACKM, bool XM, bool LM, bool WS, bool P16 = false>
 __device__ __forceinline__ void stem2_body(const StemArgs& p) {
     constexpr bool TRI = ITM > 0;
+    static_assert(!P16 || (XM && !PACK2 && NCH > 0 && ((WS && IT2_ == 1) || (!WS && IT2_ == 2))),
+                  "paired stores: a wave whose two items are the two column groups of a row tile");
     static_assert(!LM, "reserved (the limb intermediate was removed): kernel names stay 17 arguments long");
     static_assert(BF3 || !AR::fp16, "fp16 x 2: the 16-bit kernels only (its object has no fp32 products)");
     static_assert(!AR::fp16 || !TRI, "fp16 x 2: pairs and single steps");
@@ -625,6 +627,7 @@
     f32x16 axm[XM1 ? RT1 : 1];
     constexpr int NST = PACK2 ? 8 : 16;
     float2 pv[RI2 ? 1 : NST];
+    float2 pw[P16 ? NST : 1];
     float* pdst = C;
     constexpr int NSET = RI2 ? (IT2 > 1 ? 2 : 1) : 1;
     f32x16 cr[NSET][2];
@@ -642,11 +645,23 @@
             *(float2*)q = v;
         }
     };
+    auto store4 = [&](float* q, float2 v, float2 w) __attribute__((always_inline)) {
+#ifdef CTG_STEM_BOUNDS
+        if ((uint64_t)((char*)q - (char*)C) + 16 > (uint64_t)p.c_elems * 8) {
+            atomicAdd(&ctg_stem_oob<AR>[1], 1ull);
+            return;
+        }
+#endif
+        if constexpr (STEM_NT_STORES) __builtin_nontemporal_store(f32x4{v.x, v.y, w.x, w.y}, (f32x4*)q);
+        else *(f32x4*)q = f32x4{v.x, v.y, w.x, w.y};
+    };
     auto drain = [&](int lo, int hi, auto set_tag, auto scaled_tag) __attribute__((always_inline)) {
         constexpr int SET = decltype(set_tag)::value < NSET ? decltype(set_tag)::value : 0;
 #pragma unroll
         for (int i = lo; i < hi; ++i) {
-            if constexpr (RI2) {
+            if constexpr (P16) {
+                store4(pdst + 2 * out_t(i), pv[i], pw[i]);
+            } else if constexpr (RI2) {
                 float2 v;
                 v.x = cr[SET][i >> 3][2 * (i & 7)];
                 v.y = cr[SET][i >> 3][2 * (i & 7) + 1];
@@ -870,8 +885,9 @@
     auto item2 = [&](int item, int64_t c_row, auto scaled_tag, auto drain_tag, auto defer_tag)
                      __attribute__((always_inline)) {
         constexpr bool DRAIN = decltype(drain_tag)::value;
-        if constexpr (DRAIN && (K2Q == 0 || BF3)) drain(0, NST, std::integral_constant<int, 0>{}, scaled_tag);
+        if constexpr (DRAIN && !P16 && (K2Q == 0 || BF3)) drain(0, NST, std::integral_constant<int, 0>{}, scaled_tag);
         const int cg = item / n_rt2, rt2 = item - cg * n_rt2;
+        const int col = PACK2 ? (l31 & 15) : (P16 ? 64 * ((item % SW) / n_rt2) + 2 * l31 + item / SW : cg * 32 + l31);
         f32x16 cx, cy;
         if constexpr (!XM2) {
 #pragma unroll
@@ -883,12 +899,12 @@
         const float* a_base = mid + kk * PLANE + (rt2 * 32 + l31) * LD2;
         const float* bxp = b2x + cg * 32 * LDB2;
         const float* byp = PACK2 ? nullptr : b2y + cg * 32 * LDB2;
-        const int64_t c_col = oc_s[PACK2 ? (l31 & 15) : cg * 32 + l31];
+        const int64_t c_col = oc_s[col];
         const int nq = K2 >> 2;
         f32x4 af[2], bx[2], by[2];
         f32x16 cxm;
         if constexpr (XM2) {
-            const unsigned short* bR = Q2 + (cg * 32 + l31) * ROW2 + kk * 24;
+            const unsigned short* bR = Q2 + col * ROW2 + kk * 24;
             const unsigned short* bI = bR + N2 * ROW2;
             const float* aRf = mid + (rt2 * 32 + l31) * LD2 + kk * 8;
             struct Frag { bf16x8 ar[3], ai[3], br[3], bi[3]; };
@@ -1012,7 +1028,8 @@
         }
         {
             constexpr bool SC = decltype(scaled_tag)::value;
-            pdst = C + 2 * (c_row + out_lane + c_col);
+            constexpr bool SECOND = P16 && DRAIN;
+            if constexpr (!SECOND) pdst = C + 2 * (c_row + out_lane + c_col);
             if (PACK2) {
                 const bool hi = (l31 >> 4) != 0;
 #pragma unroll
@@ -1038,7 +1055,8 @@
                     v.x = SC ? xr * alpha * alpha2 : xr;
                     v.y = SC ? cy[t] * alpha * alpha2 : cy[t];
                     if constexpr (BF3) h2_vmax = fmaxf(h2_vmax, fmaxf(fabsf(v.x), fabsf(v.y)));
-                    pv[t] = v;
+                    if constexpr (SECOND) pw[t] = v;
+                    else pv[t] = v;
                 }
             }
             if constexpr (!decltype(defer_tag)::value) drain(0, NST, std::integral_constant<int, 0>{}, scaled_tag);
@@ -1084,8 +1102,8 @@
                 cy = AR::mfma(A_.ai[ta], B_.br[tb], cy);
             }
         };
-        auto emit = [&](int cg) __attribute__((always_inline)) {
-            pdst = C + 2 * (c_row + out_lane + oc_s[cg * 32 + l31]);
+        auto emit = [&](int col, auto second_tag) __attribute__((always_inline)) {
+            if constexpr (!decltype(second_tag)::value) pdst = C + 2 * (c_row + out_lane + oc_s[col]);
 #pragma unroll
             for (int t = 0; t < 16; ++t) {
                 float2 v;
@@ -1093,14 +1111,16 @@
                 v.x = SC ? xr * alpha * alpha2 : xr;
                 v.y = SC ? cy[t] * alpha * alpha2 : cy[t];
                 h2_vmax = fmaxf(h2_vmax, fmaxf(fabsf(v.x), fabsf(v.y)));
-                pv[t] = v;
+                if constexpr (decltype(second_tag)::value) pw[t] = v;
+                else pv[t] = v;
             }
         };
         static_for<0, 2>([&](auto gi) __attribute__((always_inline)) {
             constexpr int G = decltype(gi)::value;
             const int cg = cg0 + G * cgs;
-            const unsigned short* bR = Q2 + (cg * 32 + l31) * ROW2 + kk * 24;
-            if constexpr (G == 1) drain(0, NST, std::integral_constant<int, 0>{}, scaled_tag);
+            const int col = P16 ? 64 * cg0 + 2 * l31 + G : cg * 32 + l31;
+            const unsigned short* bR = Q2 + col * ROW2 + kk * 24;
+            if constexpr (G == 1 && !P16) drain(0, NST, std::integral_constant<int, 0>{}, scaled_tag);
             if constexpr (G == 0) load_a(AK[0], 0);
             load_b(BF[0], bR, 0);
             static_for<0, NC>([&](auto ci) __attribute__((always_inline)) {
@@ -1111,7 +1131,7 @@
                 }
                 mul(AK[CH], BF[CH & 1], CH == 0);
             });
-            emit(cg);
+            emit(col, std::integral_constant<bool, (P16 && G == 1)>{});
         });
     };
     f32x16 mx[TRI ? ITM : 1], my[TRI ? ITM : 1];
@@ -1248,9 +1268,9 @@
             const int64_t c_tile = tile_c(gc);
             int64_t c_rows[IT2];
             if constexpr (IT2 == 2 && XM2) {
-                if (n_rt2 <= PW) {
+                if (P16 || n_rt2 <= PW) {
                     const int nc = K2 >> 4;
-                    if (nc == 4) {
+                    if (P16 || nc == 4) {
                         item2k(std::integral_constant<int, 4>{}, wave1, item_row(wave1, c_tile), scaled_tag);
                         return;
                     }
@@ -1441,6 +1461,18 @@
 __global__ __launch_bounds__(SW * 64, 1) void stem2h_kernel(StemArgs p) {
     stem2_body<Fp16x2, PACK1, PACK2, RT1_, CS1, NCH, IT2_, BR1, K2Q, VEC, BF3, RI2, ONE, ITM, PACKM, XM, LM, WS>(p);
 }
+template <bool PACK1, bool PACK2, int RT1_, int CS1, int NCH, int IT2_, bool BR1 = false, int K2Q = 0, bool VEC = false,
+          bool BF3 = false, bool RI2 = false, bool ONE = false, int ITM = 0, bool PACKM = false, bool XM = false,
+          bool LM = false, bool WS = false>
+__global__ __launch_bounds__(SW * 64, 1) void stem2_kernel_p16(StemArgs p) {
+    stem2_body<Bf16x3, PACK1, PACK2, RT1_, CS1, NCH, IT2_, BR1, K2Q, VEC, BF3, RI2, ONE, ITM, PACKM, XM, LM, WS, true>(p);
+}
+template <bool PACK1, bool PACK2, int RT1_, int CS1, int NCH, int IT2_, bool BR1 = false, int K2Q = 0, bool VEC = false,
+          bool BF3 = false, bool RI2 = false, bool ONE = false, int ITM = 0, bool PACKM = false, bool XM = false,
+          bool LM = false, bool WS = false>
+__global__ __launch_bounds__(SW * 64, 1) void stem2h_kernel_p16(StemArgs p) {
+    stem2_body<Fp16x2, PACK1, PACK2, RT1_, CS1, NCH, IT2_, BR1, K2Q, VEC, BF3, RI2, ONE, ITM, PACKM, XM, LM, WS, true>(p);
+}
 
 #ifdef CTG_STEM_TIMELINE
 template <class AR>
@@ -1473,6 +1505,11 @@
     if constexpr (AR::fp16) return stem2h_kernel<A...>;
     else return stem2_kernel<A...>;
 }
+template <class AR, auto... A>
+static auto stem_kernel_p16() {
+    if constexpr (AR::fp16) return stem2h_kernel_p16<A...>;
+    else return stem2_kernel_p16<A...>;
+}
 
 static size_t stem2_lds_bytes(const StemArgs& p) {
     const size_t b1 = (size_t)(p.N1 == 16 ? 3 : 2) * p.N1 * (p.K1 + 4);
@@ -1494,13 +1531,35 @@
     return 4 * (b1 + (b2_in_regs ? (mid > b2 ? mid : b2) : b2 + mid)) + 8 * (size_t)p.N2;
 }
 
+static bool stem_pair16_shape(const StemArgs& p, bool ws) {
+    if (!p.pair16 || p.one || p.tri || env_on("CTG_STEM_NO_PAIR16")) return false;
+    const int n_rt2 = p.rows2 >> 5;
+    if (p.N2 != 32 * p.ng2 || n_rt2 < 1) return false;
+    if (ws) return n_rt2 == SW / 2 && p.ng2 == 2 && p.K2 == 64;
+    return n_rt2 <= SW && SW % n_rt2 == 0 && n_rt2 * p.ng2 == 2 * SW;
+}
+#ifdef CTG_STEM_PAIR16_SYM
+constexpr bool STEM_PAIR16_SYM = true;
+#else
+constexpr bool STEM_PAIR16_SYM = false;
+#endif
+static int stem_last_paired = 0;
+
 template <class AR, bool PACK1, bool PACK2, int RT1, int CS1, int NCH, int IT2, bool BR1 = false, int K2Q = 0, bool VEC = false,
           bool BF3 = false, bool RI2 = false, bool XM = false, bool WS = false>
 static hipError_t launch_stem2_t(const StemArgs& p, hipStream_t stream) {
     auto kern = stem_kernel<AR, PACK1, PACK2, RT1, CS1, NCH, IT2, BR1, K2Q, VEC, BF3, RI2, false, 0, false, XM, false, WS>();
-    static unsigned long long ready = 0;
+    static unsigned long long ready = 0, ready16 = 0;
+    bool paired = false;
+    if constexpr (BF3 && XM && !PACK2 && NCH > 0 && ((AR::fp16 && WS && IT2 == 1) || (STEM_PAIR16_SYM && !WS && IT2 == 2))) {
+        if (stem_pair16_shape(p, WS)) {
+            kern = stem_kernel_p16<AR, PACK1, PACK2, RT1, CS1, NCH, IT2, BR1, K2Q, VEC, BF3, RI2, false, 0, false, XM, false, WS>();
+            paired = true;
+        }
+    }
+    stem_last_paired = paired ? 1 : 0;
     {
-        const hipError_t e = lds_opt_in((const void*)kern, 160 * 1024, &ready);
+        const hipError_t e = lds_opt_in((const void*)kern, 160 * 1024, paired ? &ready16 : &ready);
         if (e != hipSuccess) return e;
     }
 #ifdef CTG_STEM_TIMELINE
diff --git a/cotengra_amd/runtime.py b/cotengra_amd/runtime.py
--- a/cotengra_amd/runtime.py
+++ b/cotengra_amd/runtime.py
@@ -36,6 +36,9 @@
     "ctg_exec_launch_count",
     "ctg_exec_profile_slice",
     "ctg_exec_step_kernel",
+    "ctg_exec_step_paired_stores",
+    "ctg_exec_step_stem_max",
+    "ctg_plan_stem_pair16",
     "ctg_exec_sync",
     "ctg_exec_result_ptr",
     "ctg_exec_result_stats",
@@ -145,6 +148,9 @@
         "ctg_exec_launch_count": [vp, i64p, i64p],
         "ctg_exec_profile_slice": [vp, C.c_int64, C.POINTER(C.c_float)],
         "ctg_exec_step_kernel": [vp, C.c_int64, C.c_char_p, C.c_int64],
+        "ctg_exec_step_paired_stores": [vp, C.c_int64, C.POINTER(C.c_int)],
+        "ctg_exec_step_stem_max": [vp, C.c_int64, C.c_int64, C.POINTER(C.c_float)],
+        "ctg_plan_stem_pair16": [vp, C.c_int64, C.POINTER(C.c_int)],
         "ctg_exec_sync": [vp],
         "ctg_exec_result_ptr": [vp, C.POINTER(vp)],
         "ctg_exec_result_stats": [vp, C.POINTER(C.c_double), C.POINTER(C.c_double), C.POINTER(C.c_double), i64p],
@@ -278,6 +284,15 @@
         _check(load().ctg_plan_nslices(self.handle, C.byref(n)))
         return n.value
 
+    def stem_pair16(self):
+        fn = load().ctg_plan_stem_pair16
+        out = []
+        for s in range(len(self.plan.steps)):
+            v = C.c_int()
+            _check(fn(self.handle, s, C.byref(v)))
+            out.append(bool(v.value))
+        return out
+
     def share_units(self, rank=0, world=1):
         u, g = C.c_int64(), C.c_int64()
         _check(load().ctg_plan_share_units(self.handle, int(rank), int(world), C.byref(u), C.byref(g)))
@@ -412,6 +427,20 @@
             names.append(buf.value.decode())
         return names
 
+    def step_paired_stores(self):
+        fn = load().ctg_exec_step_paired_stores
+        out = []
+        for s in range(len(self.plan.steps)):
+            v = C.c_int()
+            _check(fn(self.handle, s, C.byref(v)))
+            out.append(bool(v.value))
+        return out
+
+    def step_stem_max(self, step, z=0):
+        v = C.c_float()
+        _check(load().ctg_exec_step_stem_max(self.handle, int(step), int(z), C.byref(v)))
+        return float(v.value)
+
     def sync(self):
         _check(load().ctg_exec_sync(self.handle))
 
diff --git a/include/ctg_hip.h b/include/ctg_hip.h
--- a/include/ctg_hip.h
+++ b/include/ctg_hip.h
@@ -85,6 +85,9 @@
 int ctg_exec_profile_slice(ctg_exec* exec, int64_t slice_id, float* ms);
 
 int ctg_exec_step_kernel(ctg_exec* exec, int64_t step, char* buf, int64_t buflen);
+int ctg_exec_step_paired_stores(ctg_exec* exec, int64_t step, int* paired);
+int ctg_exec_step_stem_max(ctg_exec* exec, int64_t step, int64_t z, float* mx);
+int ctg_plan_stem_pair16(ctg_plan* plan, int64_t step, int* ok);
 
 int ctg_exec_sync(ctg_exec* exec);
 int ctg_exec_result_ptr(ctg_exec* exec, void** dev_ptr);
```

After: 174800 billion FLOP/s, median of 6. +1.1%, better.
